# zzzxxxttt/SimpleDepthEstimation

Measured on AMD Instinct MI355X. Metric: training images/sec at 192x640 bs=12/GPU, higher is better.
Workload: dtype bf16; 1 GPU; Supervised ResNet-50 (BASELINE configs[1]), bf16 storage / fp32 accumulate, bs=12/GPU, 192x640, fwd+bwd+optimizer, random-init weights; global_batch=12, parallelism=dp1, hip_graph=True, allreduce_overlap=False

## Files before the change

include/sde_hip.h:

```cpp
#ifndef SDE_HIP_H
#define SDE_HIP_H
#include <stddef.h>
#include <stdint.h>

#ifdef __cplusplus
extern "C" {
#endif

typedef void* sde_stream_t;

#define SDE_MAX_CTX 4
#define SDE_F32 0
#define SDE_BF16 1
#define SDE_F16 2

#define SDE_REDUCE_ROWS 32

#define SDE_RESIZE_BILINEAR_AC 0
#define SDE_RESIZE_NEAREST 1

const char* sde_last_error(void);
int sde_version(void);

int sde_mark_time(uint64_t* slot, sde_stream_t stream);
// ... 22 lines not shown
    float ssim_w, C1, C2;
    const float* clip_thr;
} sde_photo_desc;

int sde_photo_num_blocks(int B, int h, int w, int backward);

int sde_photo_fwd(const sde_photo_desc* d, float* const* sampled, uint8_t* sel, float* maps, float* partial, float* loss_out,
                  float loss_scale, int accumulate, sde_stream_t stream);

int sde_photo_bwd(const sde_photo_desc* d, const float* const* sampled, const uint8_t* sel, const float* gout, float gscale, float* d_depth,
                  int accumulate_depth, float* pose_partial, float* const* d_pose, int accumulate_pose, sde_stream_t stream);
int sde_photo_multi_fwd(const sde_photo_desc* d, int n, float* const* sampled, uint8_t* const* sel, float* const* partial, float* loss_out,
                        sde_stream_t stream);
int sde_photo_multi_bwd(const sde_photo_desc* d, int n, const float* const* sampled, const uint8_t* const* sel, const float* gout, float* const* d_depth,
                        float* const* pose_partial, float* const* d_pose, sde_stream_t stream);
int sde_photo_multi_pose_finalize(const sde_photo_desc* d, int n, const float* const* pose_partial, float* const* d_pose, sde_stream_t stream);

int sde_mono_loss_fwd(const sde_photo_desc* d, int n, const float* photo_w, const float* smooth_w, float* const* sampled, uint8_t* const* sel,
                      float* const* photo_partial, float* const* sm_mean_part, float* const* sm_dn, float* const* sm_loss_part, float* const* sm_s_part,
                      float* per_scale, float* totals, int* ticket, sde_stream_t stream);
int sde_mono_loss_bwd(const sde_photo_desc* d, int n, const float* photo_w, const float* smooth_w, const float* const* sampled, const uint8_t* const* sel,
                      const float* g_rec, const float* g_smooth, const float* const* sm_mean_part, const float* const* sm_dn, const float* const* sm_s_part,
                      float* const* d_depth, float* const* pose_partial, float* const* d_pose, sde_stream_t stream);
int sde_smooth_multi_bwd(const sde_photo_desc* d, int n, const float* smooth_w, const float* g_smooth, const float* const* sm_mean_part, const float* const* sm_dn,
                         const float* const* sm_s_part, float* const* d_depth, int accumulate, sde_stream_t stream);

int sde_ssim_fwd(const float* x, const float* y, int B, int C, int H, int W, float C1, float C2, float* out, sde_stream_t stream);
int sde_ssim_bwd(const float* x, const float* y, const float* gout, int B, int C, int H, int W, float C1, float C2, float* coef_ws, float* dx, float* dy,
                 sde_stream_t stream);

int sde_smooth_num_blocks(int B, int h, int w);
int sde_smooth_fwd(const float* depth, const float* img, int B, int h, int w, float* mean_part, float* dn, float* loss_part, float* s_part,
                   float* loss_out, float loss_scale, int accumulate, sde_stream_t stream);
int sde_smooth_bwd(const float* depth, const float* dn, const float* mean_part, const float* s_part, const float* gout, float gscale, int B,
                   int h, int w, float* d_depth, int accumulate, sde_stream_t stream);

int sde_silog_num_blocks(int B, int h, int w);
int sde_silog_fwd(const float* est, const float* gt, int B, int h, int w, int H, int W, float variance_focus, float* part, float* stats,
                  sde_stream_t stream);
int sde_silog_bwd(const float* est, const float* gt, const float* stats, const float* gout, float gscale, float variance_focus, int B, int h,
                  int w, int H, int W, float* d_est, int accumulate, sde_stream_t stream);
#define SDE_SILOG_MAX_SCALES 4
int sde_silog_multi_num_blocks(int B, const int* h, const int* w, int n);
int sde_silog_multi_fwd(const float* const* est, const float* gt, int B, const int* h, const int* w, const float* weight, int n, int H, int W,
                        float variance_focus, float* part, float* stats, float* total, sde_stream_t stream);
int sde_silog_multi_bwd(const float* const* est, const float* gt, const float* stats, const float* gout, float gscale, float variance_focus, int B,
                        const int* h, const int* w, const float* weight, int n, int H, int W, float* const* d_est, sde_stream_t stream);

#define SDE_SRC_PLAIN 0
#define SDE_SRC_UPCAT 1
#define SDE_SRC_ZEROINS 2
#define SDE_ACT_NONE 0
#define SDE_ACT_ELU 1
#define SDE_ACT_RELU 2

typedef struct sde_conv_desc {
    const void* x0;
    const void* x1;
    int32_t dtype;
    int32_t C0, C1, H0, W0, IH, IW, src_mode;
    int32_t KH, KW, stride, pad;
    int32_t reflect;
    int32_t Bn, OH, OW;
} sde_conv_desc;

int sde_pack_weight(const float* w, void* out, int dtype, int Cout, int Cin, int KH, int KW, int Cin_pad, int Cout_pad, int for_dgrad,
                    sde_stream_t stream);

typedef struct sde_pack_item {
    const float* src;
    void* dst_fwd;
    void* dst_dgrad;
    int32_t Cout, Cin, KH, KW, Cin_pad, Cout_pad;
    int32_t src_layout, reserved;
    int64_t end;
} sde_pack_item;
#define SDE_W_OIHW 0
#define SDE_W_OHWI 1
int sde_pack_item_blocks(int Cout_pad, int Cin_pad, int KH, int KW);
int sde_pack_weights_batched(const sde_pack_item* items_dev, int n, long total_blocks, int dtype, sde_stream_t stream);

int sde_conv_fwd(const sde_conv_desc* d, const void* w_packed, const float* bias, int act, void* y, int Cout, int ldy, float* stats,
                 sde_stream_t stream);
size_t sde_conv_fwd_ws_bytes(const sde_conv_desc* d, int ldy);
int sde_conv_fwd_ws(const sde_conv_desc* d, const void* w_packed, const float* bias, int act, void* y, int Cout, int ldy, float* stats, void* ws,
                    size_t ws_bytes, sde_stream_t stream);
int sde_conv_dgrad_bnbwd_rows(const sde_conv_desc* d, int Cout, int ldy);
int sde_conv_dgrad_bnbwd(const sde_conv_desc* d, const void* w_packed, void* gm, int Cout, int ldy, const void* bn_y, const float* bnp, float* part,
                         sde_stream_t stream);
int sde_conv_dgrad_bnbwd_res_rows(const sde_conv_desc* d, int Cout, int ldy);
int sde_conv_dgrad_bnbwd_res(const sde_conv_desc* d, const void* w_packed, void* gm, int Cout, int ldy, const void* bn_y, const float* bnp, float* part,
                             const void* res_grad, const void* bn_out, sde_stream_t stream);
int sde_conv_fwd_tiles_m(const sde_conv_desc* d, int ldy);
int sde_conv_fwd_variant(const sde_conv_desc* d, int ldy);
int sde_conv_set_halo_min_blocks(int min_blocks);
#define SDE_OPT_PGEMM 1
#define SDE_OPT_PGEMM_DEPTH 2
#define SDE_OPT_PGEMM_3X3 3
#define SDE_OPT_PGEMM_TILE 4
#define SDE_OPT_SPLITK 5
#define SDE_OPT_WGRAD_BLOCKS 6
#define SDE_OPT_WGRAD_HALO 7
#define SDE_OPT_CONV_SMALL 8
#define SDE_OPT_WGRAD_DMA 9
#define SDE_OPT_BNBWD_FUSE 10
#define SDE_OPT_CU_RESERVE 11
#define SDE_OPT_WGRAD_DMA_RING 12
#define SDE_OPT_PGEMM_PER_CU 13
int sde_conv_set_option(int key, int value);
#define SDE_KERNEL_PGEMM 1
#define SDE_KERNEL_WGRAD_DMA 2
#define SDE_KERNEL_WGRAD_HALO 3
#define SDE_KERNEL_WGRAD_STAGED 4
#define SDE_KERNEL_WGRAD_SUM 5
#define SDE_KERNEL_WGRAD_REDUCE 6
int sde_kernel_lds_bytes(int kind, int variant);

#define SDE_WGRAD_FOLD_ROWS 16
int sde_conv_wgrad_splits(const sde_conv_desc* d, int Cout);
#define SDE_WGRAD_HALO_KERNEL 1
#define SDE_WGRAD_DMA_KERNEL 2
#define SDE_WGRAD_STAGED_KERNEL 3
int sde_conv_wgrad_variant(const sde_conv_desc* d, int Cout, int ldd);
int sde_conv_wgrad(const sde_conv_desc* d, const void* dy, int Cout, int ldd, int Cin_real, float* slab, int splits, float* dw, int accumulate,
                   sde_stream_t stream);

int sde_conv_wgrad_partial(const sde_conv_desc* d, const void* dy, int Cout, int ldd, float* slab, int splits, sde_stream_t stream);
typedef struct sde_wreduce_item {
    const float* slab;
    float* dw;
    int32_t rows , Cout, KHW, Cin_pad, Cin_real;
    int32_t accumulate;
} sde_wreduce_item;
#define SDE_WREDUCE_ACCUMULATE 1
#define SDE_WREDUCE_OHWI 2
int sde_wgrad_reduce_batched(const sde_wreduce_item* items, int n, sde_stream_t stream);

int sde_prep_input(const float* img, const float* mean, const float* std_, int B, int C, int H, int W, int Cpad, int flip, int dtype, void* out,
                   sde_stream_t stream);

int sde_bn_finalize(const float* part, int tiles, int C, long count, const float* gamma, const float* beta, float* running_mean, float* running_var,
                    float momentum, float eps, float* bnp, sde_stream_t stream);
int sde_bn_eval_params(const float* gamma, const float* beta, const float* running_mean, const float* running_var, float eps, int C, float* bnp,
                       sde_stream_t stream);
int sde_bn_apply(const void* y, const float* bnp, const void* residual, int relu, long M, int C, int dtype, void* out, sde_stream_t stream);
int sde_bn_finalize_apply_ok(int tiles, int C, int dtype);
int sde_bn_set_fuse(int on);
int sde_bn_finalize_apply(const float* part, int tiles, int C, long count, const float* gamma, const float* beta, float* running_mean, float* running_var,
                          float momentum, float eps, float* bnp, const void* y, const void* residual, int relu, int dtype, void* out, sde_stream_t stream);
int sde_reduce_num_blocks(long M, int C);
int sde_bn_bwd(const void* dout, const void* dout1, const void* dout2, const void* out, const void* y, const float* bnp, const float* gamma, int relu,
               long M, int C, int dtype, float* part, float* coef, float* dgamma, float* dbeta, int accumulate_params, void* gm, void* dy,
               sde_stream_t stream);
int sde_bn_bwd_from_part(const float* part, int rows, const void* gm, const void* y, const float* bnp, long M, int C, int dtype, float* coef,
                         float* dgamma, float* dbeta, int accumulate_params, void* dy, sde_stream_t stream);

int sde_maxpool_fwd(const void* x, int B, int H, int W, int C, int dtype, void* out, uint8_t* idx, sde_stream_t stream);
int sde_maxpool_bwd(const void* dout, const uint8_t* idx, int B, int H, int W, int C, int dtype, void* dx, sde_stream_t stream);
int sde_maxpool_bwd_sum(const void* dout, const void* dout1, const uint8_t* idx, int B, int H, int W, int C, int dtype, void* dx, sde_stream_t stream);

int sde_act_bwd_bias(const void* dout, const void* out, int act, long M, int C, int dtype, void* dz, float* part, float* dbias, int Cbias, int accumulate,
                     sde_stream_t stream);
int sde_act_bwd_bias_sum(const void* dout, const void* dout1, const void* out, int act, long M, int C, int dtype, void* dz, float* part, float* dbias, int Cbias,
                         int accumulate, sde_stream_t stream);
typedef struct sde_colsum_item {
    const float* part;
    float* out;
    int32_t rows, ld, C, accumulate;
} sde_colsum_item;
int sde_colsum_finalize_batched(const sde_colsum_item* items, int n, sde_stream_t stream);

int sde_refl_fold(const void* dxp, int B, int H, int W, int C, int C0, int upcat, int dtype, void* dx0, void* dx1, sde_stream_t stream);

int sde_depth_head_fwd(const void* y, int B, int H, int W, int ld, float min_depth, float max_depth, int flip, int dtype, float* depth, sde_stream_t stream);
int sde_depth_head_bwd(const void* y, const float* ddepth, int B, int H, int W, int ld, float min_depth, float max_depth, int flip, int dtype, void* dy,
                       sde_stream_t stream);
int sde_depth_head_bias_blocks(int B, int H, int W);
int sde_depth_head_bwd_bias(const void* y, const float* ddepth, int B, int H, int W, int ld, float min_depth, float max_depth, int flip, int dtype, void* dy,
                            float* part, float* dbias, int accumulate, sde_stream_t stream);

#define SDE_GN_CHUNKS 64
int sde_gn_relu_fwd(const void* x, const float* gamma, const float* beta, int B, int HW, int C, int G, float eps, int relu, int dtype, float* part, float* gnp,
                    void* out, sde_stream_t stream);
int sde_gn_relu_bwd(const void* dout, const void* out, const void* x, const float* gnp, const float* gamma, int B, int HW, int C, int G, int relu, int dtype,
                    float* part, float* coef, float* dgamma, float* dbeta, int accumulate_params, void* dx, sde_stream_t stream);
int sde_gn_relu_res_fwd(const void* x, const void* res, const float* gamma, const float* beta, int B, int HW, int C, int G, float eps, int relu, int dtype,
                        float* part, float* gnp, void* out, sde_stream_t stream);
int sde_gn_relu_res_bwd(const void* dout, const void* out, const void* x, const void* res, const float* gnp, const float* gamma, int B, int HW, int C, int G, int relu,
                        int dtype, float* part, float* coef, float* dgamma, float* dbeta, int accumulate_params, void* dx, sde_stream_t stream);

int sde_dilate_split(const void* x, int B, int H, int W, int C, int d, int dtype, void* out, sde_stream_t stream);
int sde_dilate_merge(const void* sub, int B, int H, int W, int C, int d, int dtype, void* out, sde_stream_t stream);
int sde_upsample2_fwd(const void* x, int B, int H, int W, int C, int dtype, void* out, sde_stream_t stream);
int sde_upsample2_bwd(const void* dout, int B, int H, int W, int C, int dtype, void* dx, sde_stream_t stream);
#define SDE_CAT_MAX 6
typedef struct sde_cat_piece {
    void* p;
    int32_t C, ld, f32map, reserved;
} sde_cat_piece;
int sde_cat_fwd(const sde_cat_piece* pieces, int n, long P, int Ct, int dtype, void* out, sde_stream_t stream);
int sde_cat_bwd(const void* dout, long P, int Ct, int dtype, const sde_cat_piece* grads, int n, sde_stream_t stream);
#define SDE_STATS_ROWS 256
int sde_channel_stats_tiles(long M);
int sde_channel_stats(const void* x, long M, int C, int dtype, float* part, sde_stream_t stream);
int sde_relu_fwd(const void* x, long n, int dtype, void* y, sde_stream_t stream);
int sde_lpg_fwd(const void* y, int B, int h, int w, int ld, int r, float max_depth, int ds, int dtype, float* full, float* down, sde_stream_t stream);
int sde_lpg_bwd(const void* y, const float* dfull, const float* ddown, int B, int h, int w, int ld, int r, float max_depth, int ds, int dtype, void* dy,
                sde_stream_t stream);
int sde_sigmoid_head_fwd(const void* y, int B, int H, int W, int ld, float scale, const float* focal, float focal_div, int flip, int dtype, float* out,
                         sde_stream_t stream);
int sde_sigmoid_head_bwd(const void* y, const float* dout, int B, int H, int W, int ld, float scale, const float* focal, float focal_div, int flip, int dtype,
                         void* dy, sde_stream_t stream);


#define SDE_RLN_CHUNKS 32
int sde_randln_chunks(int HW);
int sde_randln_fwd(const void* y, const void* res, const float* gamma, const float* beta, const float* z, const float* stddev, int train, int B, int HW,
                   int C, int Cr, float eps, int relu, int dtype, float* part, float* rlnp, void* out, sde_stream_t stream);
int sde_randln_bwd(const void* d0, const void* d1, const void* d2, const void* out, const void* y, const float* rlnp, const float* gamma, int relu, int B,
                   int HW, int C, int Cr, int dtype, float* part, float* dgamma, float* dbeta, int accumulate, void* gm, void* dx, sde_stream_t stream);
int sde_bilinear2_fwd(const void* x, int B, int H, int W, int C, int dtype, void* out, sde_stream_t stream);
int sde_bilinear2_bwd(const void* dout, int B, int H, int W, int C, int dtype, void* dx, sde_stream_t stream);
int sde_softplus_head_fwd(const void* y, int B, int H, int W, int ld, int flip, int dtype, float* out, sde_stream_t stream);
int sde_softplus_head_bwd(const void* y, const float* dout, int B, int H, int W, int ld, int flip, int dtype, void* dy, sde_stream_t stream);

int sde_deconv3x3s2_fwd(const void* x, const void* w_packed, const float* bias, int act, int B, int H, int W, int C, int Cout, int ldy, int dtype,
                        void* y, sde_stream_t stream);

int sde_gconv3x3_stats_rows(int B, int H, int W, int C, int G, int stride, int dtype);
int sde_gconv3x3_fwd(const void* x, const float* w, int w_ohwi, int B, int H, int W, int C, int G, int stride, int dtype, void* y, float* stats,
                     sde_stream_t stream);
int sde_gconv3x3_dgrad(const void* dz, const float* w, int w_ohwi, int B, int H, int W, int C, int G, int stride, int dtype, void* dx,
                       sde_stream_t stream);
size_t sde_gconv3x3_wgrad_ws_bytes(int B, int H, int W, int C, int G, int stride, int dtype);
int sde_gconv3x3_wgrad(const void* x, const void* dz, int B, int H, int W, int C, int G, int stride, int dtype, float* ws, size_t ws_bytes, float* dw,
                       int flags, sde_stream_t stream);

int sde_motion_resize_cat_fwd(const float* field, int h, int w, const void* skip, int B, int H, int W, int Cs, int Cr, int Cx, int dtype, void* X,
                              float* up, sde_stream_t stream);
int sde_motion_resize_cat_bwd(const void* dX0, const void* dX1, const float* dup, int B, int H, int W, int Cx, int Cr, int Cs, int h, int w, int dtype,
                              float* dfield, void* dskip, sde_stream_t stream);
int sde_motion_tail_fwd(const void* o1, const void* o2, const float* w3, const float* up, long P, int ld, int mid, int dtype, float* out,
                        sde_stream_t stream);
int sde_motion_tail_blocks(long P, int ld, int dtype);
int sde_motion_tail_bwd(const float* dout, const void* o1, const void* o2, const float* w3, long P, int ld, int mid, int dtype, void* do1, void* do2,
                        float* part, float* dw3, sde_stream_t stream);
int sde_motion_head_blocks(long P);
int sde_motion_head_fwd(const float* field, const float* scale, const float* weight, int mask, int B, int H, int W, float* part, unsigned char* keep,
                        float* out, sde_stream_t stream);
int sde_motion_head_bwd(const float* dout, const float* field, const float* scale, const float* weight, const unsigned char* keep, int B, int H, int W,
                        float* dfield, float* part, sde_stream_t stream);
int sde_prep_input_bwd(const void* d0, const void* d1, int B, int C, int H, int W, int Cp, int dtype, float* dimg, sde_stream_t stream);

int sde_conv3d_fwd(const void* x, const float* w, const float* bias, int B, int H, int W, int D, int dtype, void* y, sde_stream_t stream);
int sde_conv3d_dgrad(const void* dy, const float* w, int B, int H, int W, int D, int dtype, void* dx, sde_stream_t stream);
int sde_conv3d_wgrad_num_blocks(int B, int H, int W, int D, int dtype);
int sde_conv3d_wgrad(const void* x, const void* dy, int B, int H, int W, int D, int dtype, float* part, float* dw, float* dbias, int accumulate,
                     sde_stream_t stream);

int sde_space_to_depth(const void* x, int B, int H, int W, int C, int dtype, void* y, sde_stream_t stream);
int sde_depth_to_space(const void* x, int B, int H, int W, int C4, int dtype, void* y, sde_stream_t stream);
int sde_concat_fwd(const void* p0, const void* p1, const float* inv, int add, int B, int H, int W, int C0, int C1, int Ct, int dtype, void* out,
                   sde_stream_t stream);
int sde_concat_bwd(const void* dout, int add, int B, int H, int W, int C0, int C1, int Ct, int dtype, void* d0, void* d1, float* d_inv, sde_stream_t stream);
int sde_inv_depth_head_fwd(const void* y, int B, int H, int W, int ld, float min_depth_head, float min_depth, float max_depth, int flip, int dtype, float* inv,
                           float* depth, sde_stream_t stream);
int sde_inv_depth_head_bwd(const void* y, const float* d_inv, const float* d_depth, int B, int H, int W, int ld, float min_depth_head, float min_depth,
                           float max_depth, int flip, int dtype, void* dy, sde_stream_t stream);

#define SDE_ADAM_MAX_SEG 8
#define SDE_GRAD_NORM_WORK 1024
typedef struct sde_adam_desc {
    long seg_end[SDE_ADAM_MAX_SEG];
    float seg_lr[SDE_ADAM_MAX_SEG], seg_wd[SDE_ADAM_MAX_SEG];
    int32_t nseg, decoupled_wd;
    float beta1, beta2, eps, bias_corr1, bias_corr2, grad_scale;
    const float* scale_state;
    double beta1_d, beta2_d;
    const float* clip_state;
} sde_adam_desc;
int sde_adam_step(float* p, const float* g, float* m, float* v, long n, const sde_adam_desc* d, sde_stream_t stream);
int sde_grad_check(const float* g, long n, float* scale_state, sde_stream_t stream);
int sde_grad_norm(const float* g, long n, float* work, float* clip_state, float grad_scale, float max_norm, sde_stream_t stream);
int sde_loss_scale_update(float* scale_state, float growth_factor, float backoff_factor, int growth_interval, sde_stream_t stream);


int sde_image_prep_u8(const uint8_t* src, int N, int Hs, int Ws, int h, int w, const int* xtab, const int* ytab, const float* jit, unsigned* lsum, float* img,
                      float* orig, sde_stream_t stream);
int sde_image_prep_u8_multi(const uint8_t* const* src, int G, int N, int Hs, int Ws, int h, int w, const int* xtab, const int* ytab, const float* jit, unsigned* lsum,
                            float* const* img, float* const* orig, sde_stream_t stream);

#define SDE_EVAL_NSUM 11
int sde_depth_metrics_num_blocks(int crop_h, int crop_w);
int sde_depth_metrics(const float* pred, int ph, int pw, const float* gt, int gh, int gw, const int* ymap, const int* xmap, int y0, int y1,
                      int x0, int x1, float min_depth, float max_depth, int gt_scale, double* part, float* med, unsigned* keys, double* out,
                      sde_stream_t stream);

int sde_depth_present(const float* pred, int N, int ph, int pw, const int* ymap, const int* xmap, int H, int W, float vmax, float gamma,
                      const uint8_t* lut, const uint8_t* frame, float* depth_full, uint16_t* depth_u16, uint8_t* canvas, sde_stream_t stream);

typedef struct sde_rgbd_desc {
    const float *frame_A, *frame_B, *depth_A, *depth_B, *K, *R, *t;
    int32_t N, H, W, ssim;
    float C1, C2;
} sde_rgbd_desc;
int sde_view_synthesis_pp(const float* img, const float* depth, const float* K, const float* R, const float* t, int B, int C, int H, int W, float* sampled,
// ... 52 lines not shown
```

simpledepthestimation_amd/csrc/nn.hip:

```cpp
#include <stdlib.h>
#include "common.h"
#include "sde_hip.h"

namespace {

template <typename T> struct VecOf;
template <> struct VecOf<float> { static constexpr int V = 4; };
template <> struct VecOf<bf16_t> { static constexpr int V = 8; };
template <> struct VecOf<half_t> { static constexpr int V = 8; };

template <typename T> __device__ __forceinline__ void load_vec(const T* p, float* v);
template <> __device__ __forceinline__ void load_vec<float>(const float* p, float* v) {
    const float4 t = *reinterpret_cast<const float4*>(p);
    v[0] = t.x; v[1] = t.y; v[2] = t.z; v[3] = t.w;
}
template <> __device__ __forceinline__ void load_vec<bf16_t>(const bf16_t* p, float* v) {
    const uint4 t = *reinterpret_cast<const uint4*>(p);
    const uint32_t w[4] = {t.x, t.y, t.z, t.w};
#pragma unroll
    for (int i = 0; i < 4; ++i) {
        v[2 * i] = __uint_as_float(w[i] << 16);
        v[2 * i + 1] = __uint_as_float(w[i] & 0xffff0000u);
    }
}
template <> __device__ __forceinline__ void load_vec<half_t>(const half_t* p, float* v) {
    typedef __attribute__((ext_vector_type(8))) _Float16 h8;
    const h8 t = *reinterpret_cast<const h8*>(p);
#pragma unroll
    for (int i = 0; i < 8; ++i) v[i] = (float)t[i];
}
template <typename T> __device__ __forceinline__ void store_vec(T* p, const float* v);
template <> __device__ __forceinline__ void store_vec<float>(float* p, const float* v) {
    *reinterpret_cast<float4*>(p) = make_float4(v[0], v[1], v[2], v[3]);
}
template <> __device__ __forceinline__ void store_vec<bf16_t>(bf16_t* p, const float* v) {
    bf16_t o[8];
#pragma unroll
    for (int i = 0; i < 8; ++i) o[i] = (bf16_t)v[i];
    *reinterpret_cast<uint4*>(p) = *reinterpret_cast<uint4*>(o);
}

template <> __device__ __forceinline__ void store_vec<half_t>(half_t* p, const float* v) {
    typedef __attribute__((ext_vector_type(8))) _Float16 h8;
    h8 o;
#pragma unroll
    for (int i = 0; i < 8; ++i) o[i] = (_Float16)v[i];
    *reinterpret_cast<h8*>(p) = o;
}

template <typename T>
__global__ void __launch_bounds__(256) prep_input_kernel(const float* __restrict__ img, const float* __restrict__ mean, const float* __restrict__ std_,
                                                         int B, int C, int H, int W, int Cpad, int flip, T* __restrict__ out) {
    const long n = (long)B * H * W;
    for (long i = (long)blockIdx.x * 256 + threadIdx.x; i < n; i += (long)gridDim.x * 256) {
        const int x = (int)(i % W), y = (int)((i / W) % H), b = (int)(i / ((long)W * H));
        const int xs = flip ? W - 1 - x : x;
        T* o = out + i * Cpad;
        for (int c = 0; c < Cpad; ++c) {
            float v = 0.f;
            if (c < C) {
                v = img[(((long)b * C + c) * H + y) * W + xs];
                if (mean) v = (v - mean[c]) / std_[c];
            }
            o[c] = (T)v;
        }
    }
}

__global__ void __launch_bounds__(1024) rows_reduce_kernel(const float* __restrict__ in, int rows, int width, int chunk, float* __restrict__ out) {
    __shared__ float sh[16][64];
    const int col = blockIdx.x * 64 + (threadIdx.x & 63), sub = threadIdx.x >> 6, ro = blockIdx.y;
    const int r0 = ro * chunk, r1 = min(rows, r0 + chunk);
    float s = 0.f;
    if (col < width)
        for (int r = r0 + sub; r < r1; r += 16) s += in[(size_t)r * width + col];
    sh[sub][threadIdx.x & 63] = s;
    __syncthreads();
    if (sub == 0 && col < width) {
        float t = 0.f;
#pragma unroll
        for (int i = 0; i < 16; ++i) t += sh[i][threadIdx.x & 63];
        out[(size_t)ro * width + col] = t;
    }
}

__device__ __forceinline__ double half_wave_sum(double v) {
#pragma unroll
    for (int o = 16; o > 0; o >>= 1) v += __shfl_xor(v, o, 64);
    return v;
}

constexpr int SLAB_T = 1024, SLAB_RL = SLAB_T / 16, SLAB_RES = SLAB_RL * 17, SLAB_SH = SLAB_RES + 16;
__device__ __forceinline__ void slab_colsum16(const float* __restrict__ part, int rows, int width, int col0, double* sh ) {
    const int rl = threadIdx.x >> 4, e = threadIdx.x & 15;
    const bool ok = col0 + e < width;
    const float* src = part + col0 + e;
    double a0 = 0, a1 = 0, a2 = 0, a3 = 0;
    int t = rl;
    if (ok) {
        for (; t + 7 * SLAB_RL < rows; t += 8 * SLAB_RL) {
            float v[8];
#pragma unroll
            for (int i = 0; i < 8; ++i) v[i] = src[(size_t)(t + i * SLAB_RL) * width];
            a0 += (double)v[0] + (double)v[4]; a1 += (double)v[1] + (double)v[5]; a2 += (double)v[2] + (double)v[6]; a3 += (double)v[3] + (double)v[7];
        }
        for (; t + 3 * SLAB_RL < rows; t += 4 * SLAB_RL) {
            const float v0 = src[(size_t)t * width], v1 = src[(size_t)(t + SLAB_RL) * width], v2 = src[(size_t)(t + 2 * SLAB_RL) * width],
                        v3 = src[(size_t)(t + 3 * SLAB_RL) * width];
            a0 += v0; a1 += v1; a2 += v2; a3 += v3;
        }
        for (; t < rows; t += SLAB_RL) a0 += src[(size_t)t * width];
    }
    sh[rl * 17 + e] = (a0 + a1) + (a2 + a3);
    __syncthreads();
    if (threadIdx.x < 16) {
        double tot = 0;
        for (int i = 0; i < SLAB_RL; ++i) tot += sh[i * 17 + threadIdx.x];
        sh[SLAB_RES + threadIdx.x] = tot;
    }
    __syncthreads();
}

__global__ void __launch_bounds__(SLAB_T) bn_finalize_kernel(const float* __restrict__ part, int tiles, int C, float count, const float* __restrict__ gamma,
                                                          const float* __restrict__ beta, float* __restrict__ rmean, float* __restrict__ rvar,
                                                          float momentum, float eps, float* __restrict__ bnp) {
    __shared__ double sh[SLAB_SH];
    slab_colsum16(part, tiles, 2 * C, blockIdx.x * 16, sh);
    const int c = blockIdx.x * 8 + threadIdx.x;
    if (threadIdx.x >= 8 || c >= C) return;
    const double s1 = sh[SLAB_RES + 2 * threadIdx.x], s2 = sh[SLAB_RES + 2 * threadIdx.x + 1];
    const double mean = s1 / count;
    double var = s2 / count - mean * mean;
    if (var < 0) var = 0;
    const float rstd = (float)(1.0 / sqrt(var + (double)eps));
    const float sc = gamma[c] * rstd;
    bnp[c] = (float)mean; bnp[C + c] = rstd; bnp[2 * C + c] = sc; bnp[3 * C + c] = beta[c] - (float)mean * sc;
    if (rmean) {
        const double unb = count > 1.f ? var * count / (count - 1.0) : var;
        rmean[c] = (1.f - momentum) * rmean[c] + momentum * (float)mean;
        rvar[c] = (1.f - momentum) * rvar[c] + momentum * (float)unb;
    }
}

__global__ void __launch_bounds__(64) bn_eval_params_kernel(const float* __restrict__ gamma, const float* __restrict__ beta,
                                                            const float* __restrict__ rmean, const float* __restrict__ rvar, float eps, int C,
                                                            float* __restrict__ bnp) {
    const int c = blockIdx.x * 64 + threadIdx.x;
    if (c >= C) return;
    const float rstd = 1.0f / sqrtf(rvar[c] + eps);
    const float sc = gamma[c] * rstd;
    bnp[c] = rmean[c]; bnp[C + c] = rstd; bnp[2 * C + c] = sc; bnp[3 * C + c] = beta[c] - rmean[c] * sc;
}

template <typename T>
__global__ void __launch_bounds__(256) bn_apply_kernel(const T* __restrict__ y, const float* __restrict__ bnp, const T* __restrict__ res, int relu,
                                                       long M, int C, T* __restrict__ out) {
    constexpr int V = VecOf<T>::V;
    const int cch = C / V;
    const long total = M * cch;
    for (long i = (long)blockIdx.x * 256 + threadIdx.x; i < total; i += (long)gridDim.x * 256) {
        const int c0 = (int)(i % cch) * V;
        float v[V], r[V];
        load_vec<T>(y + i * V, v);
        if (res) load_vec<T>(res + i * V, r);
#pragma unroll
        for (int e = 0; e < V; ++e) {
            float t = fmaf(v[e], bnp[2 * C + c0 + e], bnp[3 * C + c0 + e]);
            if (res) t += r[e];
            if (relu) t = fmaxf(t, 0.f);
            v[e] = t;
        }
        store_vec<T>(out + i * V, v);
    }
}

constexpr int BNFA_MAX_ROWS = 256;
template <typename T>
__global__ void __launch_bounds__(256) bn_finalize_apply_kernel(const float* __restrict__ part, int rows, int C, float count, const float* __restrict__ gamma,
                                                                const float* __restrict__ beta, float* __restrict__ rmean, float* __restrict__ rvar,
                                                                float momentum, float eps, float* __restrict__ bnp, const T* __restrict__ y,
                                                                const T* __restrict__ res, int relu, long M, long rows_per_wg, T* __restrict__ out) {
    constexpr int V = VecOf<T>::V;
    __shared__ double acc[8][128];
    __shared__ float ss[2][64];
    const int strip = blockIdx.x, c0 = strip * 64;
    const int tid = threadIdx.x;
    {
        const int f4 = tid & 31, rl = tid >> 5;
        const float4* src = reinterpret_cast<const float4*>(part + (size_t)c0 * 2) + f4;
        const size_t ld4 = (size_t)C / 2;
        double a[4] = {0, 0, 0, 0}, b[4] = {0, 0, 0, 0};
        int r = rl;
        for (; r + 56 < rows; r += 64) {
            float4 v[8];
#pragma unroll
            for (int i = 0; i < 8; ++i) v[i] = src[(size_t)(r + 8 * i) * ld4];
#pragma unroll
            for (int i = 0; i < 8; i += 2) {
                a[0] += v[i].x; a[1] += v[i].y; a[2] += v[i].z; a[3] += v[i].w;
                b[0] += v[i + 1].x; b[1] += v[i + 1].y; b[2] += v[i + 1].z; b[3] += v[i + 1].w;
            }
        }
        for (; r < rows; r += 8) { const float4 v = src[(size_t)r * ld4]; a[0] += v.x; a[1] += v.y; a[2] += v.z; a[3] += v.w; }
#pragma unroll
        for (int e = 0; e < 4; ++e) acc[rl][f4 * 4 + e] = a[e] + b[e];
    }
    __syncthreads();
    if (tid < 64) {
        const int c = c0 + tid;
        double s1 = 0, s2 = 0;
#pragma unroll
        for (int i = 0; i < 8; ++i) { s1 += acc[i][2 * tid]; s2 += acc[i][2 * tid + 1]; }
        const double mean = s1 / count;
        double var = s2 / count - mean * mean;
        if (var < 0) var = 0;
        const float rstd = (float)(1.0 / sqrt(var + (double)eps));
        const float sc = gamma[c] * rstd, sf = beta[c] - (float)mean * sc;
        ss[0][tid] = sc; ss[1][tid] = sf;
        if (blockIdx.y == 0) {
            bnp[c] = (float)mean; bnp[C + c] = rstd; bnp[2 * C + c] = sc; bnp[3 * C + c] = sf;
            if (rmean) {
                const double unb = count > 1.f ? var * count / (count - 1.0) : var;
                rmean[c] = (1.f - momentum) * rmean[c] + momentum * (float)mean;
                rvar[c] = (1.f - momentum) * rvar[c] + momentum * (float)unb;
            }
        }
    }
    __syncthreads();
    const int g8 = tid & 7, rl = tid >> 3;
    float sc[V], sf[V];
#pragma unroll
    for (int e = 0; e < V; ++e) { sc[e] = ss[0][g8 * V + e]; sf[e] = ss[1][g8 * V + e]; }
    const long r0 = (long)blockIdx.y * rows_per_wg, r1 = min(M, r0 + rows_per_wg);
    for (long r = r0 + rl; r < r1; r += 32) {
        const long off = r * C + c0 + g8 * V;
        float v[V], rr[V];
        load_vec<T>(y + off, v);
        if (res) load_vec<T>(res + off, rr);
#pragma unroll
        for (int e = 0; e < V; ++e) {
            float t = fmaf(v[e], sc[e], sf[e]);
            if (res) t += rr[e];
            if (relu) t = fmaxf(t, 0.f);
            v[e] = t;
        }
        store_vec<T>(out + off, v);
    }
}

template <int NV, int NT = 256>
__device__ __forceinline__ void block_group_reduce(float (&a)[NV], int cch, float* sh) {
    const int t = threadIdx.x;
#pragma unroll
    for (int e = 0; e < NV; ++e) sh[e * NT + t] = a[e];
    __syncthreads();
    if (NT > 256) {
        if (t < 256) {
            for (int r = t + 256; r < NT; r += 256)
#pragma unroll
                for (int e = 0; e < NV; ++e) a[e] += sh[e * NT + r];
#pragma unroll
            for (int e = 0; e < NV; ++e) sh[e * NT + t] = a[e];
        }
        __syncthreads();
    }
    if (t < cch) {
        for (int r = t + cch; r < 256; r += cch)
#pragma unroll
            for (int e = 0; e < NV; ++e) a[e] += sh[e * NT + r];
    }
}

template <typename T, int V>
__device__ __forceinline__ void round_vec(float* d) {
    if (sizeof(T) == 4) return;
#pragma unroll
    for (int e = 0; e < V; ++e) d[e] = (float)(T)d[e];
}

template <typename T, int V>
__device__ __forceinline__ void bn_load_dz(const T* d0, const T* d1, const T* d2, const T* out, int relu, long off, float* d, const float* yv,
                                           const float* sc, const float* sf) {
    load_vec<T>(d0 + off, d);
    if (d1) {
        float t[V];
        load_vec<T>(d1 + off, t);
#pragma unroll
        for (int e = 0; e < V; ++e) d[e] += t[e];
    }
    if (d2) {
        float t[V];
        load_vec<T>(d2 + off, t);
#pragma unroll
        for (int e = 0; e < V; ++e) d[e] += t[e];
    }
    if (relu == 1) {
        float o[V];
        load_vec<T>(out + off, o);
#pragma unroll
        for (int e = 0; e < V; ++e) d[e] = o[e] > 0.f ? d[e] : 0.f;
    } else if (relu == 2) {
#pragma unroll
        for (int e = 0; e < V; ++e) d[e] = fmaf(yv[e], sc[e], sf[e]) > 0.f ? d[e] : 0.f;
    }
}

template <typename T, int NT = 256>
__global__ void __launch_bounds__(NT) bn_bwd_reduce_kernel(const T* __restrict__ dout, const T* __restrict__ dout1, const T* __restrict__ dout2,
                                                           const T* __restrict__ out, const T* __restrict__ y,
                                                           const float* __restrict__ bnp, int relu, long M, int C, long rows_per_block,
                                                           float* __restrict__ part, T* __restrict__ gm) {
    constexpr int V = VecOf<T>::V;
    extern __shared__ float sh[];
    const int cch = C / V;
    if (NT > 256 || (cch <= 256 && 256 % cch == 0)) {
        const int col = threadIdx.x % cch, c0 = col * V;
        float mean[V], rstd[V], sc[V], sf[V], acc[2 * V];
#pragma unroll
        for (int e = 0; e < V; ++e) {
            mean[e] = bnp[c0 + e]; rstd[e] = bnp[C + c0 + e]; sc[e] = bnp[2 * C + c0 + e]; sf[e] = bnp[3 * C + c0 + e];
            acc[e] = 0.f; acc[V + e] = 0.f;
        }
        const long total = M * cch;
        for (long i = (long)blockIdx.x * NT + threadIdx.x; i < total; i += (long)gridDim.x * NT) {
            float d[V], yv[V];
            load_vec<T>(y + i * V, yv);
            bn_load_dz<T, V>(dout, dout1, dout2, out, relu, i * V, d, yv, sc, sf);
            if (gm) {
                round_vec<T, V>(d);
                store_vec<T>(gm + i * V, d);
            }
#pragma unroll
            for (int e = 0; e < V; ++e) { acc[e] += d[e]; acc[V + e] += d[e] * ((yv[e] - mean[e]) * rstd[e]); }
        }
        block_group_reduce<2 * V, NT>(acc, cch, sh);
        if (threadIdx.x < cch) {
#pragma unroll
            for (int e = 0; e < V; ++e) {
                part[((size_t)blockIdx.x * C + c0 + e) * 2] = acc[e];
                part[((size_t)blockIdx.x * C + c0 + e) * 2 + 1] = acc[V + e];
            }
        }
        return;
    }
    for (int i = threadIdx.x; i < 2 * C; i += 256) sh[i] = 0.f;
    __syncthreads();
    const long r0 = (long)blockIdx.x * rows_per_block, r1 = min(M, r0 + rows_per_block);
    const long total = (r1 - r0) * cch;
    for (long i = threadIdx.x; i < total; i += 256) {
        const int col = (int)(i % cch), c0 = col * V;
        const long off = (r0 * cch + i) * V;
        float d[V], yv[V];
        load_vec<T>(y + off, yv);
        bn_load_dz<T, V>(dout, dout1, dout2, out, relu, off, d, yv, bnp + 2 * C + c0, bnp + 3 * C + c0);
        if (gm) {
            round_vec<T, V>(d);
            store_vec<T>(gm + off, d);
        }
#pragma unroll
        for (int e = 0; e < V; ++e) {
            const float xh = (yv[e] - bnp[c0 + e]) * bnp[C + c0 + e];
            atomicAdd(&sh[c0 + e], d[e]); atomicAdd(&sh[C + c0 + e], d[e] * xh);
        }
    }
    __syncthreads();
    for (int i = threadIdx.x; i < C; i += 256) {
        part[((size_t)blockIdx.x * C + i) * 2] = sh[i];
        part[((size_t)blockIdx.x * C + i) * 2 + 1] = sh[C + i];
    }
}

__global__ void __launch_bounds__(SLAB_T) bn_bwd_finalize_kernel(const float* __restrict__ part, int nblk, int C, float count, float* __restrict__ dgamma,
                                                              float* __restrict__ dbeta, int accumulate, float* __restrict__ coef) {
    __shared__ double sh[SLAB_SH];
    slab_colsum16(part, nblk, 2 * C, blockIdx.x * 16, sh);
    const int c = blockIdx.x * 8 + threadIdx.x;
    if (threadIdx.x >= 8 || c >= C) return;
    const double s1 = sh[SLAB_RES + 2 * threadIdx.x], s2 = sh[SLAB_RES + 2 * threadIdx.x + 1];
    coef[c] = (float)(s1 / count); coef[C + c] = (float)(s2 / count);
    dgamma[c] = accumulate ? dgamma[c] + (float)s2 : (float)s2;
    dbeta[c] = accumulate ? dbeta[c] + (float)s1 : (float)s1;
}

template <typename T>
__global__ void __launch_bounds__(256) bn_bwd_apply_kernel(const T* __restrict__ dz_in, const T* __restrict__ y,
                                                           const float* __restrict__ bnp, const float* __restrict__ coef, long M, int C,
                                                           T* __restrict__ dy) {
    constexpr int V = VecOf<T>::V;
    const int cch = C / V;
    const long total = M * cch;
    for (long i = (long)blockIdx.x * 256 + threadIdx.x; i < total; i += (long)gridDim.x * 256) {
        const int c0 = (int)(i % cch) * V;
        float d[V], yv[V], g[V];
        load_vec<T>(dz_in + i * V, d);
        load_vec<T>(y + i * V, yv);
#pragma unroll
        for (int e = 0; e < V; ++e) {
            const float xh = (yv[e] - bnp[c0 + e]) * bnp[C + c0 + e];
            g[e] = bnp[2 * C + c0 + e] * (d[e] - coef[c0 + e] - xh * coef[C + c0 + e]);
        }
        store_vec<T>(dy + i * V, g);
    }
}

template <typename T>
__global__ void __launch_bounds__(256) bn_bwd_finalize_apply_kernel(const float* __restrict__ part, int rows, int C, float count, float* __restrict__ dgamma,
                                                                    float* __restrict__ dbeta, int accumulate, const T* __restrict__ dz_in,
                                                                    const T* __restrict__ y, const float* __restrict__ bnp, long M, long rows_per_wg,
                                                                    T* __restrict__ dy) {
    constexpr int V = VecOf<T>::V;
    __shared__ double acc[8][128];
    __shared__ float cf[2][64];
    const int c0 = blockIdx.x * 64, tid = threadIdx.x;
    {
        const int f4 = tid & 31, rl = tid >> 5;
        const float4* src = reinterpret_cast<const float4*>(part + (size_t)c0 * 2) + f4;
        const size_t ld4 = (size_t)C / 2;
        double a[4] = {0, 0, 0, 0}, b[4] = {0, 0, 0, 0};
        int r = rl;
        for (; r + 56 < rows; r += 64) {
            float4 v[8];
#pragma unroll
            for (int i = 0; i < 8; ++i) v[i] = src[(size_t)(r + 8 * i) * ld4];
#pragma unroll
            for (int i = 0; i < 8; i += 2) {
                a[0] += v[i].x; a[1] += v[i].y; a[2] += v[i].z; a[3] += v[i].w;
                b[0] += v[i + 1].x; b[1] += v[i + 1].y; b[2] += v[i + 1].z; b[3] += v[i + 1].w;
            }
        }
        for (; r < rows; r += 8) { const float4 v = src[(size_t)r * ld4]; a[0] += v.x; a[1] += v.y; a[2] += v.z; a[3] += v.w; }
#pragma unroll
        for (int e = 0; e < 4; ++e) acc[rl][f4 * 4 + e] = a[e] + b[e];
    }
    __syncthreads();
    if (tid < 64) {
        const int c = c0 + tid;
        double s1 = 0, s2 = 0;
#pragma unroll
        for (int i = 0; i < 8; ++i) { s1 += acc[i][2 * tid]; s2 += acc[i][2 * tid + 1]; }
        cf[0][tid] = (float)(s1 / count); cf[1][tid] = (float)(s2 / count);
        if (blockIdx.y == 0) {
            dgamma[c] = accumulate ? dgamma[c] + (float)s2 : (float)s2;
            dbeta[c] = accumulate ? dbeta[c] + (float)s1 : (float)s1;
        }
    }
    __syncthreads();
    const int g8 = tid & 7, rl = tid >> 3;
    float mean[V], rstd[V], sc[V], k1[V], k2[V];
#pragma unroll
    for (int e = 0; e < V; ++e) {
        const int c = c0 + g8 * V + e;
        mean[e] = bnp[c]; rstd[e] = bnp[C + c]; sc[e] = bnp[2 * C + c]; k1[e] = cf[0][g8 * V + e]; k2[e] = cf[1][g8 * V + e];
    }
    const long r0 = (long)blockIdx.y * rows_per_wg, r1 = min(M, r0 + rows_per_wg);
    for (long r = r0 + rl; r < r1; r += 32) {
        const long off = r * C + c0 + g8 * V;
        float d[V], yv[V], g[V];
        load_vec<T>(dz_in + off, d);
        load_vec<T>(y + off, yv);
#pragma unroll
        for (int e = 0; e < V; ++e) {
            const float xh = (yv[e] - mean[e]) * rstd[e];
            g[e] = sc[e] * (d[e] - k1[e] - xh * k2[e]);
        }
        store_vec<T>(dy + off, g);
    }
}

template <typename T>
__global__ void __launch_bounds__(256) maxpool_fwd_kernel(const T* __restrict__ x, int B, int H, int W, int C, int OH, int OW, T* __restrict__ out,
                                                          uint8_t* __restrict__ idx) {
    constexpr int V = VecOf<T>::V;
    const int cch = C / V;
    const long total = (long)B * OH * OW * cch;
    for (long i = (long)blockIdx.x * 256 + threadIdx.x; i < total; i += (long)gridDim.x * 256) {
        const int col = (int)(i % cch);
        const long pix = i / cch;
        const int ow = (int)(pix % OW), oh = (int)((pix / OW) % OH), b = (int)(pix / ((long)OW * OH));
        float best[V]; int bi[V];
#pragma unroll
        for (int e = 0; e < V; ++e) { best[e] = -INFINITY; bi[e] = 0; }
#pragma unroll
        for (int kh = 0; kh < 3; ++kh) {
            const int ih = oh * 2 - 1 + kh;
            if (ih < 0 || ih >= H) continue;
#pragma unroll
            for (int kw = 0; kw < 3; ++kw) {
                const int iw = ow * 2 - 1 + kw;
                if (iw < 0 || iw >= W) continue;
                float v[V];
                load_vec<T>(x + (((long)b * H + ih) * W + iw) * C + col * V, v);
#pragma unroll
                for (int e = 0; e < V; ++e)
                    if (v[e] > best[e] || v[e] != v[e]) { best[e] = v[e]; bi[e] = kh * 3 + kw; }
            }
        }
        store_vec<T>(out + i * V, best);
        uint8_t* ip = idx + i * V;
#pragma unroll
        for (int e = 0; e < V; ++e) ip[e] = (uint8_t)bi[e];
    }
}

template <typename T>
__global__ void __launch_bounds__(256) maxpool_bwd_kernel(const T* __restrict__ dout, const T* __restrict__ dout1, const uint8_t* __restrict__ idx, int B, int H,
                                                          int W, int C, int OH, int OW, T* __restrict__ dx) {
    constexpr int V = VecOf<T>::V;
    const int cch = C / V;
    const long total = (long)B * H * W * cch;
    for (long i = (long)blockIdx.x * 256 + threadIdx.x; i < total; i += (long)gridDim.x * 256) {
        const int col = (int)(i % cch);
        const long pix = i / cch;
        const int iw = (int)(pix % W), ih = (int)((pix / W) % H), b = (int)(pix / ((long)W * H));
        float g[V];
#pragma unroll
        for (int e = 0; e < V; ++e) g[e] = 0.f;
#pragma unroll
        for (int kh = 0; kh < 3; ++kh) {
            const int t = ih + 1 - kh;
            if (t < 0 || (t & 1)) continue;
            const int oh = t >> 1;
            if (oh >= OH) continue;
#pragma unroll
            for (int kw = 0; kw < 3; ++kw) {
                const int u = iw + 1 - kw;
                if (u < 0 || (u & 1)) continue;
                const int ow = u >> 1;
                if (ow >= OW) continue;
                const long o = ((((long)b * OH + oh) * OW + ow) * cch + col) * V;
                float d[V];
                load_vec<T>(dout + o, d);
                if (dout1) {
                    float t[V];
                    load_vec<T>(dout1 + o, t);
#pragma unroll
                    for (int e = 0; e < V; ++e) d[e] += t[e];
                }
                const uint8_t* ip = idx + o;
#pragma unroll
                for (int e = 0; e < V; ++e)
                    if (ip[e] == kh * 3 + kw) g[e] += d[e];
            }
        }
        store_vec<T>(dx + i * V, g);
    }
}

template <typename T>
__global__ void __launch_bounds__(256) act_bwd_bias_kernel(const T* __restrict__ dout, const T* __restrict__ dout1, const T* __restrict__ out, int act, long M,
                                                           int C, long rows_per_block, T* __restrict__ dz, float* __restrict__ part) {
    constexpr int V = VecOf<T>::V;
    extern __shared__ float sh[];
    const int cch = C / V;
    if (cch <= 256 && 256 % cch == 0) {
        const int col = threadIdx.x % cch, c0 = col * V;
        float acc[V];
#pragma unroll
        for (int e = 0; e < V; ++e) acc[e] = 0.f;
        const long total = M * cch;
        const long stride = (long)gridDim.x * 256;
        long i = (long)blockIdx.x * 256 + threadIdx.x;
        for (; i + 3 * stride < total; i += 4 * stride) {
            float d[4][V], o[4][V];
#pragma unroll
            for (int u = 0; u < 4; ++u) load_vec<T>(dout + (i + u * stride) * V, d[u]);
            if (dout1) {
#pragma unroll
                for (int u = 0; u < 4; ++u) load_vec<T>(dout1 + (i + u * stride) * V, o[u]);
#pragma unroll
                for (int u = 0; u < 4; ++u)
#pragma unroll
                    for (int e = 0; e < V; ++e) d[u][e] += o[u][e];
            }
            if (act != SDE_ACT_NONE) {
#pragma unroll
                for (int u = 0; u < 4; ++u) load_vec<T>(out + (i + u * stride) * V, o[u]);
#pragma unroll
                for (int u = 0; u < 4; ++u)
#pragma unroll
                    for (int e = 0; e < V; ++e) {
                        if (act == SDE_ACT_ELU) d[u][e] = o[u][e] > 0.f ? d[u][e] : d[u][e] * (o[u][e] + 1.0f);
                        else d[u][e] = o[u][e] > 0.f ? d[u][e] : 0.f;
                    }
            }
#pragma unroll
            for (int u = 0; u < 4; ++u) {
                if (dz) store_vec<T>(dz + (i + u * stride) * V, d[u]);
#pragma unroll
                for (int e = 0; e < V; ++e) acc[e] += d[u][e];
            }
        }
        for (; i < total; i += stride) {
            float d[V], o[V];
            load_vec<T>(dout + i * V, d);
            if (dout1) {
                load_vec<T>(dout1 + i * V, o);
#pragma unroll
                for (int e = 0; e < V; ++e) d[e] += o[e];
            }
            if (act != SDE_ACT_NONE) {
                load_vec<T>(out + i * V, o);
#pragma unroll
                for (int e = 0; e < V; ++e) {
                    if (act == SDE_ACT_ELU) d[e] = o[e] > 0.f ? d[e] : d[e] * (o[e] + 1.0f);
                    else d[e] = o[e] > 0.f ? d[e] : 0.f;
                }
            }
            if (dz) store_vec<T>(dz + i * V, d);
#pragma unroll
            for (int e = 0; e < V; ++e) acc[e] += d[e];
        }
        if (part) {
            block_group_reduce<V>(acc, cch, sh);
            if (threadIdx.x < cch)
#pragma unroll
                for (int e = 0; e < V; ++e) part[(size_t)blockIdx.x * C + c0 + e] = acc[e];
        }
        return;
    }
    if (part) {
        for (int i = threadIdx.x; i < C; i += 256) sh[i] = 0.f;
        __syncthreads();
    }
    const long r0 = (long)blockIdx.x * rows_per_block, r1 = min(M, r0 + rows_per_block);
    const long total = (r1 - r0) * cch;
    for (long i = threadIdx.x; i < total; i += 256) {
        const int c0 = (int)(i % cch) * V;
        const long off = (r0 * cch + i) * V;
        float d[V], o[V];
        load_vec<T>(dout + off, d);
        if (dout1) {
            load_vec<T>(dout1 + off, o);
#pragma unroll
            for (int e = 0; e < V; ++e) d[e] += o[e];
        }
        if (act != SDE_ACT_NONE) {
            load_vec<T>(out + off, o);
#pragma unroll
            for (int e = 0; e < V; ++e) {
                if (act == SDE_ACT_ELU) d[e] = o[e] > 0.f ? d[e] : d[e] * (o[e] + 1.0f);
                else if (act == SDE_ACT_RELU) d[e] = o[e] > 0.f ? d[e] : 0.f;
            }
        }
        if (dz) store_vec<T>(dz + off, d);
        if (part) {
#pragma unroll
            for (int e = 0; e < V; ++e) atomicAdd(&sh[c0 + e], d[e]);
        }
    }
    if (part) {
        __syncthreads();
        for (int i = threadIdx.x; i < C; i += 256) part[(size_t)blockIdx.x * C + i] = sh[i];
    }
}

__global__ void __launch_bounds__(SLAB_T) colsum_finalize_kernel(const float* __restrict__ part, int nblk, int ld, int C, float* __restrict__ out, int accumulate) {
    __shared__ double sh[SLAB_SH];
    slab_colsum16(part, nblk, ld, blockIdx.x * 16, sh);
    const int c = blockIdx.x * 16 + threadIdx.x;
    if (threadIdx.x >= 16 || c >= C) return;
    const double sv = sh[SLAB_RES + threadIdx.x];
    out[c] = accumulate ? out[c] + (float)sv : (float)sv;
}

constexpr int COLSUM_MAX_ITEMS = 64;
struct ColsumBatch {
    const float* part[COLSUM_MAX_ITEMS];
    float* out[COLSUM_MAX_ITEMS];
    int rows[COLSUM_MAX_ITEMS], ld[COLSUM_MAX_ITEMS], C[COLSUM_MAX_ITEMS], accumulate[COLSUM_MAX_ITEMS];
    int first[COLSUM_MAX_ITEMS + 1];
    int n;
};
__global__ void __launch_bounds__(SLAB_T) colsum_finalize_batched_kernel(const ColsumBatch b) {
    __shared__ double sh[SLAB_SH];
    int k = 0;
    while (k + 1 < b.n && (int)blockIdx.x >= b.first[k + 1]) ++k;
    const int col0 = ((int)blockIdx.x - b.first[k]) * 16;
    slab_colsum16(b.part[k], b.rows[k], b.ld[k], col0, sh);
    const int c = col0 + threadIdx.x;
    if (threadIdx.x >= 16 || c >= b.C[k]) return;
    const double sv = sh[SLAB_RES + threadIdx.x];
    float* out = b.out[k];
    out[c] = b.accumulate[k] ? out[c] + (float)sv : (float)sv;
}

template <typename T>
__device__ __forceinline__ void fold_at(const T* __restrict__ dxp, int b, int h, int w, int H, int W, int C, int c0, float* g) {
    constexpr int V = VecOf<T>::V;
#pragma unroll
    for (int e = 0; e < V; ++e) g[e] = 0.f;
    int hs[3], ws[3], nh = 0, nw = 0;
    hs[nh++] = h + 1;
    if (h == 1) hs[nh++] = 0;
    if (h == H - 2) hs[nh++] = H + 1;
    ws[nw++] = w + 1;
    if (w == 1) ws[nw++] = 0;
    if (w == W - 2) ws[nw++] = W + 1;
// ... 367 lines not shown
            s2 += part[((size_t)q * C + c) * 2 + 1];
        }
        s1 = wave_sum_f64(s1); s2 = wave_sum_f64(s2);
        if (threadIdx.x == 0) {
            dgamma[c] = accumulate ? dgamma[c] + (float)s2 : (float)s2;
            dbeta[c] = accumulate ? dbeta[c] + (float)s1 : (float)s1;
        }
    }
}

template <typename T>
__global__ void __launch_bounds__(256) gn_bwd_apply_kernel(const T* __restrict__ dout, const T* __restrict__ out, const T* __restrict__ x, const T* __restrict__ res,
                                                           const float* __restrict__ gnp, const float* __restrict__ coef, const float* __restrict__ gamma,
                                                           int B, int HW, int C, int G, int relu, T* __restrict__ dx) {
    constexpr int V = VecOf<T>::V;
    const int cch = C / V, cpg = C / G;
    const long total = (long)B * HW * cch;
    for (long i = (long)blockIdx.x * 256 + threadIdx.x; i < total; i += (long)gridDim.x * 256) {
        const int c0 = (int)(i % cch) * V, b = (int)(i / ((long)HW * cch));
        float d[V], o[V], xv[V];
        load_vec<T>(dout + i * V, d);
        if (relu) load_vec<T>(out + i * V, o);
        load_vec<T>(x + i * V, xv);
        if (res) {
            float rr[V];
            load_vec<T>(res + i * V, rr);
#pragma unroll
            for (int e = 0; e < V; ++e) xv[e] += rr[e];
        }
#pragma unroll
        for (int e = 0; e < V; ++e) {
            const size_t gi = ((size_t)b * G + (c0 + e) / cpg) * 2;
            float de = d[e];
            if (relu) de = gn_act_grad(de, o[e], relu);
            const float xh = (xv[e] - gnp[gi]) * gnp[gi + 1];
            d[e] = gnp[gi + 1] * (gamma[c0 + e] * de - coef[gi] - xh * coef[gi + 1]);
        }
        store_vec<T>(dx + i * V, d);
    }
}

__global__ void __launch_bounds__(256) adam_kernel(float* __restrict__ p, const float* __restrict__ g, float* __restrict__ m, float* __restrict__ v, long n,
                                                   const sde_adam_desc d) {
    float gs = d.grad_scale;
    float bc1 = d.bias_corr1, bc2 = d.bias_corr2;
    if (d.scale_state) {
        if (d.scale_state[1] != 0.f) return;
        gs /= d.scale_state[0];
        const double t = (double)d.scale_state[3] + 1.0;
        bc1 = (float)(1.0 - pow(d.beta1_d, t));
        bc2 = (float)(1.0 - pow(d.beta2_d, t));
    }
    if (d.clip_state) gs *= d.clip_state[1];
    const float beta1 = d.beta1, beta2 = d.beta2, rbc2 = 1.0f / sqrtf(bc2);
    for (long i = (long)blockIdx.x * 256 + threadIdx.x; i < n; i += (long)gridDim.x * 256) {
        int s = 0;
        while (s < d.nseg - 1 && i >= d.seg_end[s]) ++s;
        const float lr = d.seg_lr[s], wd = d.seg_wd[s];
        float gi = g[i] * gs, pi = p[i];
        if (d.decoupled_wd) pi *= (1.0f - lr * wd);
        else gi += wd * pi;
        const float mi = beta1 * m[i] + (1.0f - beta1) * gi;
        const float vi = beta2 * v[i] + (1.0f - beta2) * gi * gi;
        m[i] = mi; v[i] = vi;
        const float denom = sqrtf(vi) * rbc2 + d.eps;
        p[i] = pi - (lr / bc1) * (mi / denom);
    }
}

__global__ void __launch_bounds__(256) grad_check_kernel(const float4* __restrict__ g4, long n4, const float* __restrict__ tail, int ntail, float* __restrict__ state) {
    bool bad = false;
    for (long i = (long)blockIdx.x * 256 + threadIdx.x; i < n4; i += (long)gridDim.x * 256) {
        const float4 q = g4[i];
        const float t = fabsf(q.x) + fabsf(q.y) + fabsf(q.z) + fabsf(q.w);
        bad |= !(t <= 3.0e38f);
    }
    if (blockIdx.x == 0 && (int)threadIdx.x < ntail) bad |= !(fabsf(tail[threadIdx.x]) <= 3.0e38f);
    if (__any(bad) && (threadIdx.x & 63) == 0) state[1] = 1.0f;
}

__global__ void loss_scale_update_kernel(float* __restrict__ state, float growth, float backoff, int interval) {
    if (threadIdx.x != 0 || blockIdx.x != 0) return;
    if (state[1] != 0.f) { state[0] *= backoff; state[2] = 0.f; }
    else {
        state[3] += 1.f;
        const float t = state[2] + 1.f;
        if (t >= (float)interval) { state[0] *= growth; state[2] = 0.f; } else state[2] = t;
    }
    state[1] = 0.f;
}

__global__ void __launch_bounds__(256) grad_norm_partial_kernel(const float4* __restrict__ g4, long n4, const float* __restrict__ tail, int ntail, float* __restrict__ work) {
    __shared__ float red[16];
    float sx = 0.f, sy = 0.f, sz = 0.f, sw = 0.f;
    for (long i = (long)blockIdx.x * 256 + threadIdx.x; i < n4; i += (long)gridDim.x * 256) {
        const float4 q = g4[i];
        sx = fmaf(q.x, q.x, sx); sy = fmaf(q.y, q.y, sy); sz = fmaf(q.z, q.z, sz); sw = fmaf(q.w, q.w, sw);
    }
    float s = (sx + sy) + (sz + sw);
    if (blockIdx.x == 0 && (int)threadIdx.x < ntail) s = fmaf(tail[threadIdx.x], tail[threadIdx.x], s);
    s = sde_block_sum(s, red);
    if (threadIdx.x == 0) work[blockIdx.x] = s;
}

__global__ void __launch_bounds__(256) grad_norm_finalize_kernel(const float* __restrict__ work, int nwork, float grad_scale, float max_norm, float* __restrict__ clip_state) {
    __shared__ float red[16];
    float s = 0.f;
    for (int i = threadIdx.x; i < nwork; i += 256) s += work[i];
    s = sde_block_sum(s, red);
    if (threadIdx.x == 0) {
        const float total = grad_scale * sqrtf(s);
        float coef = max_norm / (total + 1e-6f);
        if (coef > 1.0f) coef = 1.0f;
        clip_state[0] = total;
        clip_state[1] = coef;
    }
}

const float* pre_reduce(const float* part, int& rows, int width, hipStream_t s) {
    constexpr int thr = 4096;
    if (rows <= thr) return part;
    float* out = const_cast<float*>(part) + (size_t)rows * width;
    const int chunk = (rows + SDE_REDUCE_ROWS - 1) / SDE_REDUCE_ROWS;
    const int rows_out = (rows + chunk - 1) / chunk;
    hipLaunchKernelGGL(rows_reduce_kernel, dim3((width + 63) / 64, rows_out), dim3(1024), 0, s, part, rows, width, chunk, out);
    rows = rows_out;
    return out;
}

int grid_for(long n_items) {
    long nb = (n_items + 255) / 256;
    if (nb < 1) nb = 1;
    if (nb > 8192) nb = 8192;
    return (int)nb;
}

}

#define DISPATCH_T(dtype, CALL_F32, CALL_BF16, CALL_F16) \
    do {                                        \
        if ((dtype) == SDE_BF16) { CALL_BF16; }  \
        else if ((dtype) == SDE_F16) { CALL_F16; } \
        else { CALL_F32; }                      \
    } while (0)

extern "C" {

int sde_prep_input(const float* img, const float* mean, const float* std_, int B, int C, int H, int W, int Cpad, int flip, int dtype, void* out,
                   sde_stream_t stream) {
    SDE_CHECK_ARG(img && out && B > 0 && C > 0 && H > 0 && W > 0 && Cpad >= C, "sde_prep_input: bad argument");
    SDE_CHECK_ARG((mean == nullptr) == (std_ == nullptr), "sde_prep_input: mean/std must both be given or both be null");
    hipStream_t s = (hipStream_t)stream;
    const int nb = grid_for((long)B * H * W);
    DISPATCH_T(dtype, hipLaunchKernelGGL(prep_input_kernel<float>, dim3(nb), dim3(256), 0, s, img, mean, std_, B, C, H, W, Cpad, flip, (float*)out),
               hipLaunchKernelGGL(prep_input_kernel<bf16_t>, dim3(nb), dim3(256), 0, s, img, mean, std_, B, C, H, W, Cpad, flip, (bf16_t*)out),
               hipLaunchKernelGGL(prep_input_kernel<half_t>, dim3(nb), dim3(256), 0, s, img, mean, std_, B, C, H, W, Cpad, flip, (half_t*)out));
    SDE_CHECK_LAUNCH("sde_prep_input");
    return SDE_OK;
}

int sde_bn_finalize(const float* part, int tiles, int C, long count, const float* gamma, const float* beta, float* running_mean, float* running_var,
                    float momentum, float eps, float* bnp, sde_stream_t stream) {
    SDE_CHECK_ARG(part && gamma && beta && bnp && tiles > 0 && C > 0 && count > 0, "sde_bn_finalize: bad argument");
    int rows = tiles;
    const float* src = pre_reduce(part, rows, 2 * C, (hipStream_t)stream);
    hipLaunchKernelGGL(bn_finalize_kernel, dim3(sde_cdiv(C, 8)), dim3(SLAB_T), 0, (hipStream_t)stream, src, rows, C, (float)count, gamma, beta, running_mean,
                       running_var, momentum, eps, bnp);
    SDE_CHECK_LAUNCH("sde_bn_finalize");
    return SDE_OK;
}

static int g_bn_fuse = 1;
static int g_bn_wide = 1;
int sde_bn_set_fuse(int on) {
    const int old = g_bn_fuse ? (g_bn_wide ? 1 : 2) : 0;
    g_bn_fuse = on ? 1 : 0;
    g_bn_wide = on == 1;
    return old;
}

int sde_bn_finalize_apply_ok(int tiles, int C, int dtype) { return SDE_IS16(dtype) && C % 64 == 0 && tiles >= 1 && tiles <= BNFA_MAX_ROWS; }

int sde_bn_finalize_apply(const float* part, int tiles, int C, long count, const float* gamma, const float* beta, float* running_mean, float* running_var,
                          float momentum, float eps, float* bnp, const void* y, const void* residual, int relu, int dtype, void* out, sde_stream_t stream) {
    SDE_CHECK_ARG(part && gamma && beta && bnp && y && out && count > 0, "sde_bn_finalize_apply: bad argument");
    SDE_CHECK_ARG(sde_bn_finalize_apply_ok(tiles, C, dtype), "sde_bn_finalize_apply: needs a 16-bit type, C %% 64 == 0 and <= %d slab rows (tiles=%d C=%d)",
                  BNFA_MAX_ROWS, tiles, C);
    const long M = count;
    const int strips = C / 64;
    long chunks = (1024 + strips - 1) / strips;
    long rpw = (M + chunks - 1) / chunks;
    rpw = (rpw + 31) / 32 * 32;
    if (rpw < 32) rpw = 32;
    chunks = (M + rpw - 1) / rpw;
    const dim3 grid((unsigned)strips, (unsigned)chunks);
    hipStream_t s = (hipStream_t)stream;
    if (dtype == SDE_BF16)
        hipLaunchKernelGGL(bn_finalize_apply_kernel<bf16_t>, grid, dim3(256), 0, s, part, tiles, C, (float)count, gamma, beta, running_mean, running_var, momentum, eps,
                           bnp, (const bf16_t*)y, (const bf16_t*)residual, relu, M, rpw, (bf16_t*)out);
    else
        hipLaunchKernelGGL(bn_finalize_apply_kernel<half_t>, grid, dim3(256), 0, s, part, tiles, C, (float)count, gamma, beta, running_mean, running_var, momentum, eps,
                           bnp, (const half_t*)y, (const half_t*)residual, relu, M, rpw, (half_t*)out);
    SDE_CHECK_LAUNCH("sde_bn_finalize_apply");
    return SDE_OK;
}

int sde_bn_eval_params(const float* gamma, const float* beta, const float* running_mean, const float* running_var, float eps, int C, float* bnp,
                       sde_stream_t stream) {
    SDE_CHECK_ARG(gamma && beta && running_mean && running_var && bnp && C > 0, "sde_bn_eval_params: bad argument");
    hipLaunchKernelGGL(bn_eval_params_kernel, dim3(sde_cdiv(C, 64)), dim3(64), 0, (hipStream_t)stream, gamma, beta, running_mean, running_var, eps, C, bnp);
    SDE_CHECK_LAUNCH("sde_bn_eval_params");
    return SDE_OK;
}

int sde_bn_apply(const void* y, const float* bnp, const void* residual, int relu, long M, int C, int dtype, void* out, sde_stream_t stream) {
    const int V = SDE_IS16(dtype) ? 8 : 4;
    SDE_CHECK_ARG(y && bnp && out && M > 0 && C > 0 && C % V == 0, "sde_bn_apply: bad argument (C=%d)", C);
    hipStream_t s = (hipStream_t)stream;
    const int nb = grid_for(M * (C / V));
    DISPATCH_T(dtype, hipLaunchKernelGGL(bn_apply_kernel<float>, dim3(nb), dim3(256), 0, s, (const float*)y, bnp, (const float*)residual, relu, M, C, (float*)out),
               hipLaunchKernelGGL(bn_apply_kernel<bf16_t>, dim3(nb), dim3(256), 0, s, (const bf16_t*)y, bnp, (const bf16_t*)residual, relu, M, C, (bf16_t*)out),
               hipLaunchKernelGGL(bn_apply_kernel<half_t>, dim3(nb), dim3(256), 0, s, (const half_t*)y, bnp, (const half_t*)residual, relu, M, C, (half_t*)out));
    SDE_CHECK_LAUNCH("sde_bn_apply");
    return SDE_OK;
}

int sde_reduce_num_blocks(long M, int C) {
    constexpr long cap = 1024;
    long nb = (M * (long)C / 8 + 1023) / 1024;
    if (nb > cap) nb = cap;
    if (nb < 1) nb = 1;
    return (int)nb;
}

int sde_bn_bwd(const void* dout, const void* dout1, const void* dout2, const void* out, const void* y, const float* bnp, const float* gamma, int relu,
               long M, int C, int dtype, float* part, float* coef, float* dgamma, float* dbeta, int accumulate_params, void* gm, void* dy,
               sde_stream_t stream) {
    const int V = SDE_IS16(dtype) ? 8 : 4;
    SDE_CHECK_ARG(dout && y && bnp && part && coef && dgamma && dbeta && dy && M > 0 && C > 0 && C % V == 0, "sde_bn_bwd: bad argument");
    if (relu && !out) relu = 2;
    SDE_CHECK_ARG(gm || (!relu && !dout1 && !dout2), "sde_bn_bwd: a masked or summed gradient needs the gm buffer");
    SDE_CHECK_ARG(dout1 || !dout2, "sde_bn_bwd: dout2 without dout1");
    (void)gamma;
    hipStream_t s = (hipStream_t)stream;
    int nblk = sde_reduce_num_blocks(M, C);
    const long rpb = (M + nblk - 1) / nblk;
    const size_t lds = (2 * (size_t)C > 256 * 16 ? 2 * (size_t)C : 256 * 16) * sizeof(float);
    const int cch = C / V;
    const bool wide = g_bn_fuse && g_bn_wide && SDE_IS16(dtype) && C % 64 == 0 && nblk > BNFA_MAX_ROWS && cch <= 256 && 256 % cch == 0;
    if (wide) {
        nblk = (nblk + 3) / 4;
        if (dtype == SDE_BF16)
            hipLaunchKernelGGL((bn_bwd_reduce_kernel<bf16_t, 1024>), dim3(nblk), dim3(1024), 1024 * 16 * sizeof(float), s, (const bf16_t*)dout, (const bf16_t*)dout1,
                               (const bf16_t*)dout2, (const bf16_t*)out, (const bf16_t*)y, bnp, relu, M, C, rpb, part, (bf16_t*)gm);
        else
            hipLaunchKernelGGL((bn_bwd_reduce_kernel<half_t, 1024>), dim3(nblk), dim3(1024), 1024 * 16 * sizeof(float), s, (const half_t*)dout, (const half_t*)dout1,
                               (const half_t*)dout2, (const half_t*)out, (const half_t*)y, bnp, relu, M, C, rpb, part, (half_t*)gm);
    } else
    DISPATCH_T(dtype,
               hipLaunchKernelGGL(bn_bwd_reduce_kernel<float>, dim3(nblk), dim3(256), lds, s, (const float*)dout, (const float*)dout1, (const float*)dout2, (const float*)out, (const float*)y, bnp, relu, M, C, rpb, part, (float*)gm),
               hipLaunchKernelGGL(bn_bwd_reduce_kernel<bf16_t>, dim3(nblk), dim3(256), lds, s, (const bf16_t*)dout, (const bf16_t*)dout1, (const bf16_t*)dout2, (const bf16_t*)out, (const bf16_t*)y, bnp, relu, M, C, rpb, part, (bf16_t*)gm),
               hipLaunchKernelGGL(bn_bwd_reduce_kernel<half_t>, dim3(nblk), dim3(256), lds, s, (const half_t*)dout, (const half_t*)dout1, (const half_t*)dout2, (const half_t*)out, (const half_t*)y, bnp, relu, M, C, rpb, part, (half_t*)gm));
    SDE_CHECK_LAUNCH("sde_bn_bwd/reduce");
    const void* dz = gm ? gm : dout;
    if (g_bn_fuse && SDE_IS16(dtype) && C % 64 == 0 && nblk <= BNFA_MAX_ROWS) {
        const int strips = C / 64;
        long chunks = (1024 + strips - 1) / strips;
        long rpw = (M + chunks - 1) / chunks;
        rpw = (rpw + 31) / 32 * 32;
        chunks = (M + rpw - 1) / rpw;
        const dim3 grid((unsigned)strips, (unsigned)chunks);
        if (dtype == SDE_BF16)
            hipLaunchKernelGGL(bn_bwd_finalize_apply_kernel<bf16_t>, grid, dim3(256), 0, s, part, nblk, C, (float)M, dgamma, dbeta, accumulate_params, (const bf16_t*)dz,
                               (const bf16_t*)y, bnp, M, rpw, (bf16_t*)dy);
        else
            hipLaunchKernelGGL(bn_bwd_finalize_apply_kernel<half_t>, grid, dim3(256), 0, s, part, nblk, C, (float)M, dgamma, dbeta, accumulate_params, (const half_t*)dz,
                               (const half_t*)y, bnp, M, rpw, (half_t*)dy);
        SDE_CHECK_LAUNCH("sde_bn_bwd/finalize+apply");
        return SDE_OK;
    }
    int rows = nblk;
    const float* src = pre_reduce(part, rows, 2 * C, s);
    hipLaunchKernelGGL(bn_bwd_finalize_kernel, dim3(sde_cdiv(C, 8)), dim3(SLAB_T), 0, s, src, rows, C, (float)M, dgamma, dbeta, accumulate_params, coef);
    SDE_CHECK_LAUNCH("sde_bn_bwd/finalize");
    const int nb = grid_for(M * (C / V));
    DISPATCH_T(dtype,
               hipLaunchKernelGGL(bn_bwd_apply_kernel<float>, dim3(nb), dim3(256), 0, s, (const float*)dz, (const float*)y, bnp, coef, M, C, (float*)dy),
               hipLaunchKernelGGL(bn_bwd_apply_kernel<bf16_t>, dim3(nb), dim3(256), 0, s, (const bf16_t*)dz, (const bf16_t*)y, bnp, coef, M, C, (bf16_t*)dy),
               hipLaunchKernelGGL(bn_bwd_apply_kernel<half_t>, dim3(nb), dim3(256), 0, s, (const half_t*)dz, (const half_t*)y, bnp, coef, M, C, (half_t*)dy));
    SDE_CHECK_LAUNCH("sde_bn_bwd/apply");
    return SDE_OK;
}

int sde_bn_bwd_from_part(const float* part, int rows, const void* gm, const void* y, const float* bnp, long M, int C, int dtype, float* coef,
                         float* dgamma, float* dbeta, int accumulate_params, void* dy, sde_stream_t stream) {
    const int V = SDE_IS16(dtype) ? 8 : 4;
    SDE_CHECK_ARG(part && gm && y && bnp && coef && dgamma && dbeta && dy && rows > 0 && M > 0 && C > 0 && C % V == 0, "sde_bn_bwd_from_part: bad argument");
    hipStream_t s = (hipStream_t)stream;
    if (g_bn_fuse && SDE_IS16(dtype) && C % 64 == 0 && rows <= BNFA_MAX_ROWS) {
        const int strips = C / 64;
        long chunks = (1024 + strips - 1) / strips;
        long rpw = (M + chunks - 1) / chunks;
        rpw = (rpw + 31) / 32 * 32;
        chunks = (M + rpw - 1) / rpw;
        const dim3 grid((unsigned)strips, (unsigned)chunks);
        if (dtype == SDE_BF16)
            hipLaunchKernelGGL(bn_bwd_finalize_apply_kernel<bf16_t>, grid, dim3(256), 0, s, part, rows, C, (float)M, dgamma, dbeta, accumulate_params, (const bf16_t*)gm,
                               (const bf16_t*)y, bnp, M, rpw, (bf16_t*)dy);
        else
            hipLaunchKernelGGL(bn_bwd_finalize_apply_kernel<half_t>, grid, dim3(256), 0, s, part, rows, C, (float)M, dgamma, dbeta, accumulate_params, (const half_t*)gm,
                               (const half_t*)y, bnp, M, rpw, (half_t*)dy);
        SDE_CHECK_LAUNCH("sde_bn_bwd_from_part/finalize+apply");
        return SDE_OK;
    }
    int r = rows;
    const float* src = pre_reduce(part, r, 2 * C, s);
    hipLaunchKernelGGL(bn_bwd_finalize_kernel, dim3(sde_cdiv(C, 8)), dim3(SLAB_T), 0, s, src, r, C, (float)M, dgamma, dbeta, accumulate_params, coef);
    SDE_CHECK_LAUNCH("sde_bn_bwd_from_part/finalize");
    const int nb = grid_for(M * (C / V));
    DISPATCH_T(dtype,
               hipLaunchKernelGGL(bn_bwd_apply_kernel<float>, dim3(nb), dim3(256), 0, s, (const float*)gm, (const float*)y, bnp, coef, M, C, (float*)dy),
               hipLaunchKernelGGL(bn_bwd_apply_kernel<bf16_t>, dim3(nb), dim3(256), 0, s, (const bf16_t*)gm, (const bf16_t*)y, bnp, coef, M, C, (bf16_t*)dy),
               hipLaunchKernelGGL(bn_bwd_apply_kernel<half_t>, dim3(nb), dim3(256), 0, s, (const half_t*)gm, (const half_t*)y, bnp, coef, M, C, (half_t*)dy));
    SDE_CHECK_LAUNCH("sde_bn_bwd_from_part/apply");
    return SDE_OK;
}

int sde_maxpool_fwd(const void* x, int B, int H, int W, int C, int dtype, void* out, uint8_t* idx, sde_stream_t stream) {
    const int V = SDE_IS16(dtype) ? 8 : 4;
    SDE_CHECK_ARG(x && out && idx && B > 0 && H > 1 && W > 1 && C % V == 0, "sde_maxpool_fwd: bad argument");
    const int OH = (H + 2 - 3) / 2 + 1, OW = (W + 2 - 3) / 2 + 1;
    hipStream_t s = (hipStream_t)stream;
    const int nb = grid_for((long)B * OH * OW * (C / V));
    DISPATCH_T(dtype, hipLaunchKernelGGL(maxpool_fwd_kernel<float>, dim3(nb), dim3(256), 0, s, (const float*)x, B, H, W, C, OH, OW, (float*)out, idx),
               hipLaunchKernelGGL(maxpool_fwd_kernel<bf16_t>, dim3(nb), dim3(256), 0, s, (const bf16_t*)x, B, H, W, C, OH, OW, (bf16_t*)out, idx),
               hipLaunchKernelGGL(maxpool_fwd_kernel<half_t>, dim3(nb), dim3(256), 0, s, (const half_t*)x, B, H, W, C, OH, OW, (half_t*)out, idx));
    SDE_CHECK_LAUNCH("sde_maxpool_fwd");
    return SDE_OK;
}

int sde_maxpool_bwd(const void* dout, const uint8_t* idx, int B, int H, int W, int C, int dtype, void* dx, sde_stream_t stream) {
    return sde_maxpool_bwd_sum(dout, nullptr, idx, B, H, W, C, dtype, dx, stream);
}

int sde_maxpool_bwd_sum(const void* dout, const void* dout1, const uint8_t* idx, int B, int H, int W, int C, int dtype, void* dx, sde_stream_t stream) {
    const int V = SDE_IS16(dtype) ? 8 : 4;
    SDE_CHECK_ARG(dout && idx && dx && B > 0 && H > 1 && W > 1 && C % V == 0, "sde_maxpool_bwd: bad argument");
    const int OH = (H + 2 - 3) / 2 + 1, OW = (W + 2 - 3) / 2 + 1;
    hipStream_t s = (hipStream_t)stream;
    const int nb = grid_for((long)B * H * W * (C / V));
    DISPATCH_T(dtype, hipLaunchKernelGGL(maxpool_bwd_kernel<float>, dim3(nb), dim3(256), 0, s, (const float*)dout, (const float*)dout1, idx, B, H, W, C, OH, OW, (float*)dx),
               hipLaunchKernelGGL(maxpool_bwd_kernel<bf16_t>, dim3(nb), dim3(256), 0, s, (const bf16_t*)dout, (const bf16_t*)dout1, idx, B, H, W, C, OH, OW, (bf16_t*)dx),
               hipLaunchKernelGGL(maxpool_bwd_kernel<half_t>, dim3(nb), dim3(256), 0, s, (const half_t*)dout, (const half_t*)dout1, idx, B, H, W, C, OH, OW, (half_t*)dx));
    SDE_CHECK_LAUNCH("sde_maxpool_bwd");
    return SDE_OK;
}

int sde_act_bwd_bias(const void* dout, const void* out, int act, long M, int C, int dtype, void* dz, float* part, float* dbias, int Cbias, int accumulate,
                     sde_stream_t stream) {
    return sde_act_bwd_bias_sum(dout, nullptr, out, act, M, C, dtype, dz, part, dbias, Cbias, accumulate, stream);
}

int sde_act_bwd_bias_sum(const void* dout, const void* dout1, const void* out, int act, long M, int C, int dtype, void* dz, float* part, float* dbias, int Cbias,
                         int accumulate, sde_stream_t stream) {
    const int V = SDE_IS16(dtype) ? 8 : 4;
    SDE_CHECK_ARG(dout && M > 0 && C > 0 && C % V == 0, "sde_act_bwd_bias: bad argument");
    SDE_CHECK_ARG(act == SDE_ACT_NONE || out, "sde_act_bwd_bias: activation backward needs the saved output");
    SDE_CHECK_ARG((dbias == nullptr) || (part && Cbias > 0 && Cbias <= C), "sde_act_bwd_bias: bias gradient needs a partial slab");
    hipStream_t s = (hipStream_t)stream;
    const int nblk = sde_reduce_num_blocks(M, C);
    const long rpb = (M + nblk - 1) / nblk;
    float* p = part;
    const size_t lds = ((size_t)C > 256 * 8 ? (size_t)C : 256 * 8) * sizeof(float);
    DISPATCH_T(dtype,
               hipLaunchKernelGGL(act_bwd_bias_kernel<float>, dim3(nblk), dim3(256), lds, s, (const float*)dout, (const float*)dout1, (const float*)out, act, M, C, rpb, (float*)dz, p),
               hipLaunchKernelGGL(act_bwd_bias_kernel<bf16_t>, dim3(nblk), dim3(256), lds, s, (const bf16_t*)dout, (const bf16_t*)dout1, (const bf16_t*)out, act, M, C, rpb, (bf16_t*)dz, p),
               hipLaunchKernelGGL(act_bwd_bias_kernel<half_t>, dim3(nblk), dim3(256), lds, s, (const half_t*)dout, (const half_t*)dout1, (const half_t*)out, act, M, C, rpb, (half_t*)dz, p));
    SDE_CHECK_LAUNCH("sde_act_bwd_bias");
    if (dbias) {
        int rows = nblk;
        const float* src = pre_reduce(part, rows, C, s);
        hipLaunchKernelGGL(colsum_finalize_kernel, dim3(sde_cdiv(Cbias, 16)), dim3(SLAB_T), 0, s, src, rows, C, Cbias, dbias, accumulate);
        SDE_CHECK_LAUNCH("sde_act_bwd_bias/finalize");
    }
    return SDE_OK;
}

int sde_colsum_finalize_batched(const sde_colsum_item* items, int n, sde_stream_t stream) {
    SDE_CHECK_ARG(items && n >= 0, "sde_colsum_finalize_batched: bad argument");
    for (int base = 0; base < n; base += COLSUM_MAX_ITEMS) {
        ColsumBatch b;
        b.n = n - base < COLSUM_MAX_ITEMS ? n - base : COLSUM_MAX_ITEMS;
        b.first[0] = 0;
        for (int k = 0; k < COLSUM_MAX_ITEMS; ++k) {
            const bool on = k < b.n;
            const sde_colsum_item* it = on ? items + base + k : nullptr;
            SDE_CHECK_ARG(!on || (it->part && it->out && it->rows >= 1 && it->rows <= 4096 && it->C >= 1 && it->C <= it->ld),
                          "sde_colsum_finalize_batched: item %d: bad slab (rows=%d ld=%d C=%d)", base + k, on ? it->rows : 0, on ? it->ld : 0, on ? it->C : 0);
            b.part[k] = on ? it->part : nullptr; b.out[k] = on ? it->out : nullptr;
            b.rows[k] = on ? it->rows : 0; b.ld[k] = on ? it->ld : 0; b.C[k] = on ? it->C : 0; b.accumulate[k] = on ? it->accumulate : 0;
            b.first[k + 1] = b.first[k] + (on ? sde_cdiv(it->C, 16) : 0);
        }
        if (b.first[b.n] == 0) continue;
        hipLaunchKernelGGL(colsum_finalize_batched_kernel, dim3(b.first[b.n]), dim3(SLAB_T), 0, (hipStream_t)stream, b);
        SDE_CHECK_LAUNCH("sde_colsum_finalize_batched");
    }
    return SDE_OK;
}

int sde_refl_fold(const void* dxp, int B, int H, int W, int C, int C0, int upcat, int dtype, void* dx0, void* dx1, sde_stream_t stream) {
    const int V = SDE_IS16(dtype) ? 8 : 4;
    SDE_CHECK_ARG(dxp && dx0 && B > 0 && H >= 2 && W >= 2 && C % V == 0, "sde_refl_fold: bad argument (B=%d H=%d W=%d C=%d)", B, H, W, C);
    SDE_CHECK_ARG(!upcat || (C0 > 0 && C0 <= C && C0 % V == 0 && H % 2 == 0 && W % 2 == 0 && (C0 == C || dx1)), "sde_refl_fold: bad upcat argument");
    hipStream_t s = (hipStream_t)stream;
    const long items = upcat ? (long)B * (H / 2) * (W / 2) * (C0 / V) + (long)B * H * W * ((C - C0) / V) : (long)B * H * W * (C / V);
    const int nb = grid_for(items);
    DISPATCH_T(dtype, hipLaunchKernelGGL(refl_fold_kernel<float>, dim3(nb), dim3(256), 0, s, (const float*)dxp, B, H, W, C, C0, upcat, (float*)dx0, (float*)dx1),
               hipLaunchKernelGGL(refl_fold_kernel<bf16_t>, dim3(nb), dim3(256), 0, s, (const bf16_t*)dxp, B, H, W, C, C0, upcat, (bf16_t*)dx0, (bf16_t*)dx1),
               hipLaunchKernelGGL(refl_fold_kernel<half_t>, dim3(nb), dim3(256), 0, s, (const half_t*)dxp, B, H, W, C, C0, upcat, (half_t*)dx0, (half_t*)dx1));
    SDE_CHECK_LAUNCH("sde_refl_fold");
    return SDE_OK;
}

int sde_depth_head_fwd(const void* y, int B, int H, int W, int ld, float min_depth, float max_depth, int flip, int dtype, float* depth, sde_stream_t stream) {
    SDE_CHECK_ARG(y && depth && B > 0 && H > 0 && W > 0 && ld > 0 && min_depth > 0 && max_depth > min_depth, "sde_depth_head_fwd: bad argument");
    hipStream_t s = (hipStream_t)stream;
    const float mind = 1.0f / max_depth, maxd = 1.0f / min_depth;
    const int nb = grid_for((long)B * H * W);
    DISPATCH_T(dtype, hipLaunchKernelGGL(depth_head_fwd_kernel<float>, dim3(nb), dim3(256), 0, s, (const float*)y, B, H, W, ld, mind, maxd, flip, depth),
               hipLaunchKernelGGL(depth_head_fwd_kernel<bf16_t>, dim3(nb), dim3(256), 0, s, (const bf16_t*)y, B, H, W, ld, mind, maxd, flip, depth),
               hipLaunchKernelGGL(depth_head_fwd_kernel<half_t>, dim3(nb), dim3(256), 0, s, (const half_t*)y, B, H, W, ld, mind, maxd, flip, depth));
    SDE_CHECK_LAUNCH("sde_depth_head_fwd");
    return SDE_OK;
}

int sde_depth_head_bwd(const void* y, const float* ddepth, int B, int H, int W, int ld, float min_depth, float max_depth, int flip, int dtype, void* dy,
                       sde_stream_t stream) {
    return sde_depth_head_bwd_bias(y, ddepth, B, H, W, ld, min_depth, max_depth, flip, dtype, dy, nullptr, nullptr, 0, stream);
}

int sde_depth_head_bias_blocks(int B, int H, int W) { return grid_for((long)B * H * W); }

int sde_depth_head_bwd_bias(const void* y, const float* ddepth, int B, int H, int W, int ld, float min_depth, float max_depth, int flip, int dtype, void* dy,
                            float* part, float* dbias, int accumulate, sde_stream_t stream) {
    SDE_CHECK_ARG(y && ddepth && dy && B > 0 && H > 0 && W > 0 && ld > 0, "sde_depth_head_bwd: bad argument");
    SDE_CHECK_ARG((part == nullptr) == (dbias == nullptr), "sde_depth_head_bwd_bias: the bias gradient needs both the partial buffer and the output");
    hipStream_t s = (hipStream_t)stream;
    const float mind = 1.0f / max_depth, maxd = 1.0f / min_depth;
    const int nb = grid_for((long)B * H * W);
    DISPATCH_T(dtype, hipLaunchKernelGGL(depth_head_bwd_kernel<float>, dim3(nb), dim3(256), 0, s, (const float*)y, ddepth, B, H, W, ld, mind, maxd, flip, (float*)dy, part),
               hipLaunchKernelGGL(depth_head_bwd_kernel<bf16_t>, dim3(nb), dim3(256), 0, s, (const bf16_t*)y, ddepth, B, H, W, ld, mind, maxd, flip, (bf16_t*)dy, part),
               hipLaunchKernelGGL(depth_head_bwd_kernel<half_t>, dim3(nb), dim3(256), 0, s, (const half_t*)y, ddepth, B, H, W, ld, mind, maxd, flip, (half_t*)dy, part));
    SDE_CHECK_LAUNCH("sde_depth_head_bwd");
    if (dbias) {
        hipLaunchKernelGGL(head_bias_finalize_kernel, dim3(1), dim3(256), 0, s, part, nb, dbias, accumulate);
        SDE_CHECK_LAUNCH("sde_depth_head_bwd_bias/finalize");
    }
    return SDE_OK;
}

int sde_gn_relu_fwd(const void* x, const float* gamma, const float* beta, int B, int HW, int C, int G, float eps, int relu, int dtype, float* part, float* gnp,
                    void* out, sde_stream_t stream) {
    return sde_gn_relu_res_fwd(x, nullptr, gamma, beta, B, HW, C, G, eps, relu, dtype, part, gnp, out, stream);
}

static bool gn_vector_path(int C, int dtype) { const int V = SDE_IS16(dtype) ? 8 : 4; return C % V == 0 && 256 % (C / V) == 0; }

int sde_gn_relu_res_fwd(const void* x, const void* res, const float* gamma, const float* beta, int B, int HW, int C, int G, float eps, int relu, int dtype,
                        float* part, float* gnp, void* out, sde_stream_t stream) {
    SDE_CHECK_ARG(x && gamma && beta && part && gnp && out && B > 0 && HW > 0 && C > 0 && G > 0 && C % G == 0, "sde_gn_relu_fwd: bad argument");
    SDE_CHECK_ARG(C % (SDE_IS16(dtype) ? 8 : 4) == 0, "sde_gn_relu_fwd: C=%d must be a multiple of the 16-byte group", C);
    SDE_CHECK_ARG(!res || gn_vector_path(C, dtype), "sde_gn_relu_res_fwd: the residual form needs C / (16-byte group) to divide 256 (C=%d)", C);
    hipStream_t s = (hipStream_t)stream;
    const size_t lds = 2 * (size_t)C * sizeof(float);
    DISPATCH_T(dtype, hipLaunchKernelGGL(gn_stats_kernel<float>, dim3(GN_CHUNKS, B), dim3(256), lds, s, (const float*)x, (const float*)res, HW, C, part),
               hipLaunchKernelGGL(gn_stats_kernel<bf16_t>, dim3(GN_CHUNKS, B), dim3(256), lds, s, (const bf16_t*)x, (const bf16_t*)res, HW, C, part),
               hipLaunchKernelGGL(gn_stats_kernel<half_t>, dim3(GN_CHUNKS, B), dim3(256), lds, s, (const half_t*)x, (const half_t*)res, HW, C, part));
    SDE_CHECK_LAUNCH("sde_gn_relu_fwd/stats");
    hipLaunchKernelGGL(gn_finalize_kernel, dim3(B * G), dim3(64), 0, s, part, B, C, G, HW, eps, gnp);
    SDE_CHECK_LAUNCH("sde_gn_relu_fwd/finalize");
    const int nb = grid_for((long)B * HW * (C / (SDE_IS16(dtype) ? 8 : 4)));
    DISPATCH_T(dtype, hipLaunchKernelGGL(gn_apply_kernel<float>, dim3(nb), dim3(256), 0, s, (const float*)x, (const float*)res, gnp, gamma, beta, B, HW, C, G, relu, (float*)out),
               hipLaunchKernelGGL(gn_apply_kernel<bf16_t>, dim3(nb), dim3(256), 0, s, (const bf16_t*)x, (const bf16_t*)res, gnp, gamma, beta, B, HW, C, G, relu, (bf16_t*)out),
               hipLaunchKernelGGL(gn_apply_kernel<half_t>, dim3(nb), dim3(256), 0, s, (const half_t*)x, (const half_t*)res, gnp, gamma, beta, B, HW, C, G, relu, (half_t*)out));
    SDE_CHECK_LAUNCH("sde_gn_relu_fwd/apply");
    return SDE_OK;
}

int sde_gn_relu_bwd(const void* dout, const void* out, const void* x, const float* gnp, const float* gamma, int B, int HW, int C, int G, int relu, int dtype,
                    float* part, float* coef, float* dgamma, float* dbeta, int accumulate_params, void* dx, sde_stream_t stream) {
    return sde_gn_relu_res_bwd(dout, out, x, nullptr, gnp, gamma, B, HW, C, G, relu, dtype, part, coef, dgamma, dbeta, accumulate_params, dx, stream);
}

int sde_gn_relu_res_bwd(const void* dout, const void* out, const void* x, const void* res, const float* gnp, const float* gamma, int B, int HW, int C, int G, int relu,
                        int dtype, float* part, float* coef, float* dgamma, float* dbeta, int accumulate_params, void* dx, sde_stream_t stream) {
    SDE_CHECK_ARG(dout && out && x && gnp && gamma && part && coef && dgamma && dbeta && dx && C % G == 0, "sde_gn_relu_bwd: bad argument");
    SDE_CHECK_ARG(!res || gn_vector_path(C, dtype), "sde_gn_relu_res_bwd: the residual form needs C / (16-byte group) to divide 256 (C=%d)", C);
    SDE_CHECK_ARG(C % (SDE_IS16(dtype) ? 8 : 4) == 0, "sde_gn_relu_bwd: C=%d must be a multiple of the 16-byte group", C);
    hipStream_t s = (hipStream_t)stream;
    const size_t lds = 2 * (size_t)C * sizeof(float);
    DISPATCH_T(dtype,
               hipLaunchKernelGGL(gn_bwd_stats_kernel<float>, dim3(GN_CHUNKS, B), dim3(256), lds, s, (const float*)dout, (const float*)out, (const float*)x, (const float*)res, gnp, HW, C, G, relu, part),
               hipLaunchKernelGGL(gn_bwd_stats_kernel<bf16_t>, dim3(GN_CHUNKS, B), dim3(256), lds, s, (const bf16_t*)dout, (const bf16_t*)out, (const bf16_t*)x, (const bf16_t*)res, gnp, HW, C, G, relu, part),
               hipLaunchKernelGGL(gn_bwd_stats_kernel<half_t>, dim3(GN_CHUNKS, B), dim3(256), lds, s, (const half_t*)dout, (const half_t*)out, (const half_t*)x, (const half_t*)res, gnp, HW, C, G, relu, part));
    SDE_CHECK_LAUNCH("sde_gn_relu_bwd/stats");
    hipLaunchKernelGGL(gn_bwd_finalize_kernel, dim3(B * G + C), dim3(64), 0, s, part, gamma, B, C, G, HW, coef, dgamma, dbeta, accumulate_params);
// ... 54 lines not shown
```

simpledepthestimation_amd/hip/nn.py:

```python
import contextlib
import ctypes
import functools
import os
import weakref
from collections import namedtuple
from ctypes import POINTER, Structure, c_float, c_int, c_int32, c_long, c_void_p

import torch

from . import lib as L

SRC_PLAIN, SRC_UPCAT, SRC_ZEROINS = 0, 1, 2
REDUCE_ROWS = 32
ACT_NONE, ACT_ELU, ACT_RELU = 0, 1, 2


class ConvDesc(Structure):
    _fields_ = [("x0", c_void_p), ("x1", c_void_p), ("dtype", c_int32), ("C0", c_int32), ("C1", c_int32), ("H0", c_int32), ("W0", c_int32),
                ("IH", c_int32), ("IW", c_int32), ("src_mode", c_int32), ("KH", c_int32), ("KW", c_int32), ("stride", c_int32), ("pad", c_int32),
                ("reflect", c_int32), ("Bn", c_int32), ("OH", c_int32), ("OW", c_int32)]


_P, _I, _F, _LG = c_void_p, c_int, c_float, c_long
L.register_protos({
    "sde_pack_weight": ([_P, _P, _I, _I, _I, _I, _I, _I, _I, _I, _P], c_int),
    "sde_pack_weights_batched": ([_P, _I, _LG, _I, _P], c_int),
    "sde_pack_item_blocks": ([_I, _I, _I, _I], c_int),
    "sde_conv_fwd": ([POINTER(ConvDesc), _P, _P, _I, _P, _I, _I, _P, _P], c_int),
    "sde_conv_fwd_tiles_m": ([POINTER(ConvDesc), _I], c_int),
    "sde_conv_fwd_ws_bytes": ([POINTER(ConvDesc), _I], ctypes.c_size_t),
    "sde_conv_fwd_ws": ([POINTER(ConvDesc), _P, _P, _I, _P, _I, _I, _P, _P, ctypes.c_size_t, _P], c_int),
    "sde_conv_fwd_variant": ([POINTER(ConvDesc), _I], c_int),
    "sde_conv_dgrad_bnbwd_rows": ([POINTER(ConvDesc), _I, _I], c_int),
    "sde_conv_dgrad_bnbwd": ([POINTER(ConvDesc), _P, _P, _I, _I, _P, _P, _P, _P], c_int),
    "sde_conv_dgrad_bnbwd_res_rows": ([POINTER(ConvDesc), _I, _I], c_int),
    "sde_conv_dgrad_bnbwd_res": ([POINTER(ConvDesc), _P, _P, _I, _I, _P, _P, _P, _P, _P, _P], c_int),
    "sde_bn_bwd_from_part": ([_P, _I, _P, _P, _P, _LG, _I, _I, _P, _P, _P, _I, _P, _P], c_int),
    "sde_conv_set_halo_min_blocks": ([_I], c_int),
    "sde_conv_set_option": ([_I, _I], c_int),
    "sde_kernel_lds_bytes": ([_I, _I], c_int),
    "sde_conv_wgrad_splits": ([POINTER(ConvDesc), _I], c_int),
    "sde_conv_wgrad_variant": ([POINTER(ConvDesc), _I, _I], c_int),
    "sde_conv_wgrad": ([POINTER(ConvDesc), _P, _I, _I, _I, _P, _I, _P, _I, _P], c_int),
    "sde_conv_wgrad_partial": ([POINTER(ConvDesc), _P, _I, _I, _P, _I, _P], c_int),
    "sde_wgrad_reduce_batched": ([_P, _I, _P], c_int),
    "sde_colsum_finalize_batched": ([_P, _I, _P], c_int),
    "sde_prep_input": ([_P, _P, _P, _I, _I, _I, _I, _I, _I, _I, _P, _P], c_int),
    "sde_bn_finalize": ([_P, _I, _I, _LG, _P, _P, _P, _P, _F, _F, _P, _P], c_int),
    "sde_bn_eval_params": ([_P, _P, _P, _P, _F, _I, _P, _P], c_int),
    "sde_bn_apply": ([_P, _P, _P, _I, _LG, _I, _I, _P, _P], c_int),
    "sde_bn_finalize_apply_ok": ([_I, _I, _I], c_int),
    "sde_bn_set_fuse": ([_I], c_int),
    "sde_bn_finalize_apply": ([_P, _I, _I, _LG, _P, _P, _P, _P, _F, _F, _P, _P, _P, _I, _I, _P, _P], c_int),
    "sde_reduce_num_blocks": ([_LG, _I], c_int),
    "sde_bn_bwd": ([_P, _P, _P, _P, _P, _P, _P, _I, _LG, _I, _I, _P, _P, _P, _P, _I, _P, _P, _P], c_int),
    "sde_maxpool_fwd": ([_P, _I, _I, _I, _I, _I, _P, _P, _P], c_int),
    "sde_depth_head_bias_blocks": ([_I, _I, _I], c_int),
    "sde_depth_head_bwd_bias": ([_P, _P, _I, _I, _I, _I, _F, _F, _I, _I, _P, _P, _P, _I, _P], c_int),
    "sde_maxpool_bwd": ([_P, _P, _I, _I, _I, _I, _I, _P, _P], c_int),
    "sde_maxpool_bwd_sum": ([_P, _P, _P, _I, _I, _I, _I, _I, _P, _P], c_int),
    "sde_act_bwd_bias": ([_P, _P, _I, _LG, _I, _I, _P, _P, _P, _I, _I, _P], c_int),
    "sde_act_bwd_bias_sum": ([_P, _P, _P, _I, _LG, _I, _I, _P, _P, _P, _I, _I, _P], c_int),
    "sde_refl_fold": ([_P, _I, _I, _I, _I, _I, _I, _I, _P, _P, _P], c_int),
    "sde_depth_head_fwd": ([_P, _I, _I, _I, _I, _F, _F, _I, _I, _P, _P], c_int),
    "sde_depth_head_bwd": ([_P, _P, _I, _I, _I, _I, _F, _F, _I, _I, _P, _P], c_int),
    "sde_gn_relu_fwd": ([_P, _P, _P, _I, _I, _I, _I, _F, _I, _I, _P, _P, _P, _P], c_int),
    "sde_gn_relu_bwd": ([_P, _P, _P, _P, _P, _I, _I, _I, _I, _I, _I, _P, _P, _P, _P, _I, _P, _P], c_int),
    "sde_gn_relu_res_fwd": ([_P, _P, _P, _P, _I, _I, _I, _I, _F, _I, _I, _P, _P, _P, _P], c_int),
    "sde_gn_relu_res_bwd": ([_P, _P, _P, _P, _P, _P, _I, _I, _I, _I, _I, _I, _P, _P, _P, _P, _I, _P, _P], c_int),
    "sde_space_to_depth": ([_P, _I, _I, _I, _I, _I, _P, _P], c_int),
    "sde_depth_to_space": ([_P, _I, _I, _I, _I, _I, _P, _P], c_int),
    "sde_concat_fwd": ([_P, _P, _P, _I, _I, _I, _I, _I, _I, _I, _I, _P, _P], c_int),
    "sde_concat_bwd": ([_P, _I, _I, _I, _I, _I, _I, _I, _I, _P, _P, _P, _P], c_int),
    "sde_inv_depth_head_fwd": ([_P, _I, _I, _I, _I, _F, _F, _F, _I, _I, _P, _P, _P], c_int),
    "sde_inv_depth_head_bwd": ([_P, _P, _P, _I, _I, _I, _I, _F, _F, _F, _I, _I, _P, _P], c_int),
    "sde_conv3d_fwd": ([_P, _P, _P, _I, _I, _I, _I, _I, _P, _P], c_int),
    "sde_conv3d_dgrad": ([_P, _P, _I, _I, _I, _I, _I, _P, _P], c_int),
    "sde_conv3d_wgrad_num_blocks": ([_I, _I, _I, _I, _I], c_int),
    "sde_conv3d_wgrad": ([_P, _P, _I, _I, _I, _I, _I, _P, _P, _P, _I, _P], c_int),
    "sde_adam_step": ([_P, _P, _P, _P, _LG, _P, _P], c_int),
    "sde_grad_check": ([_P, _LG, _P, _P], c_int),
    "sde_grad_norm": ([_P, _LG, _P, _P, _F, _F, _P], c_int),
    "sde_loss_scale_update": ([_P, _F, _F, _I, _P], c_int),
})


OPT_PGEMM, OPT_PGEMM_DEPTH, OPT_PGEMM_3X3, OPT_PGEMM_TILE, OPT_SPLITK, OPT_WGRAD_BLOCKS, OPT_WGRAD_HALO, OPT_CONV_SMALL, OPT_WGRAD_DMA, OPT_BNBWD_FUSE, OPT_CU_RESERVE = 1, 2, 3, 4, 5, 6, 7, 8, 9, 10, 11
OPT_WGRAD_DMA_RING, OPT_PGEMM_PER_CU = 12, 13
KERNEL_PGEMM, KERNEL_WGRAD_DMA, KERNEL_WGRAD_HALO, KERNEL_WGRAD_STAGED, KERNEL_WGRAD_SUM, KERNEL_WGRAD_REDUCE = 1, 2, 3, 4, 5, 6


def set_option(key, value):
    old = L.lib().sde_conv_set_option(int(key), int(value))
    if old < 0:
        raise L.SdeHipError(f"sde_conv_set_option({key}, {value}) failed: {L.lib().sde_last_error().decode()}")
    return old


def kernel_lds_bytes(kind, variant=0):
    n = L.lib().sde_kernel_lds_bytes(int(kind), int(variant))
    if n < 0:
        raise L.SdeHipError(f"sde_kernel_lds_bytes({kind}, {variant}): bad kind / variant")
    return n


WGRAD_HALO_KERNEL, WGRAD_DMA_KERNEL, WGRAD_STAGED_KERNEL = 1, 2, 3


def dtype_code(dt):
    if dt == torch.float32:
        return L.F32
    if dt == torch.bfloat16:
        return L.BF16
    if dt == torch.float16:
        return L.F16
    raise L.SdeHipError(f"unsupported activation dtype {dt}")


def vec_of(dt):
    return 4 if dt == torch.float32 else 8


def pad_to(c, v):
    return (c + v - 1) // v * v


def is_ohwi(t):
    return t.dim() == 4 and not t.is_contiguous() and t.permute(0, 2, 3, 1).is_contiguous()


def _dense(t):
    return t.is_contiguous() or is_ohwi(t)


def _grad_slot(p):
    g = p.grad if (p is not None and p.is_leaf) else None
    if g is not None and g.dtype == torch.float32 and _dense(g) and g.shape == p.shape:
        return g
    return None


def _f32(t):
    if t.dtype != torch.float32:
        raise L.SdeHipError("parameters must be float32")
    return t.contiguous()


def aliases(out, n):
    return out if n == 1 else (out,) + tuple(out.view(out.shape) for _ in range(n - 1))


def fan_in(douts, slots):
    grads = [g.contiguous() for g in douts if g is not None]
    if not grads:
        return ()
    for g in grads[slots:]:
        grads[slots - 1] = grads[slots - 1] + g
    return tuple(grads[:slots]) + (None,) * (slots - len(grads))


def pack_weight(w, dtype, cin_pad, cout_pad, for_dgrad=False):
    w = _f32(w)
    Cout, Cin, KH, KW = w.shape
    shape = (cin_pad, KH, KW, cout_pad) if for_dgrad else (cout_pad, KH, KW, cin_pad)
    out = torch.empty(shape, device=w.device, dtype=dtype)
    L.check(L.lib().sde_pack_weight(L.ptr(w), L.ptr(out), dtype_code(dtype), Cout, Cin, KH, KW, cin_pad, cout_pad, int(for_dgrad), L.stream()),
            "sde_pack_weight")
    return out


def _desc(x0, x1, src_mode, KH, KW, stride, pad, reflect, IH, IW, OH, OW):
    d = ConvDesc()
    B, H0, W0, C0 = x0.shape
    d.x0 = x0.data_ptr(); d.x1 = x1.data_ptr() if x1 is not None else 0
    d.dtype = dtype_code(x0.dtype)
    d.C0, d.C1, d.H0, d.W0, d.IH, d.IW = C0, (x1.shape[3] if x1 is not None else 0), H0, W0, IH, IW
    d.src_mode, d.KH, d.KW, d.stride, d.pad, d.reflect = src_mode, KH, KW, stride, pad, int(reflect)
    d.Bn, d.OH, d.OW = B, OH, OW
    return d


_timed = L.timed


def conv_raw(d, x_dtype, w_packed, bias, act, Cout, ldy, want_stats, device, kind="igemm_fwd", flops=0.0):
    y = torch.empty(d.Bn, d.OH, d.OW, ldy, device=device, dtype=x_dtype)
    stats, tiles = None, 0
    lib = L.lib()
    if want_stats:
        tiles = lib.sde_conv_fwd_tiles_m(ctypes.byref(d), ldy)
        stats = torch.empty(tiles + REDUCE_ROWS, Cout, 2, device=device, dtype=torch.float32)
    variant = lib.sde_conv_fwd_variant(ctypes.byref(d), ldy) if L.PROFILE is not None else 0
    meta = None
    if L.PROFILE is not None:
        esz = 4 if x_dtype == torch.float32 else 2
        meta = dict(M=d.Bn * d.OH * d.OW, N=ldy, K=d.KH * d.KW * (d.C0 + d.C1), k=d.KH, s=d.stride, mode=d.src_mode,
                    bytes=esz * (d.Bn * d.H0 * d.W0 * d.C0 + d.Bn * d.IH * d.IW * d.C1 + d.Bn * d.OH * d.OW * ldy))
    ws_bytes = lib.sde_conv_fwd_ws_bytes(ctypes.byref(d), ldy)
    ws = torch.empty(ws_bytes // 4, device=device, dtype=torch.float32) if ws_bytes else None
    _timed(kind, flops, variant, lambda: L.check(lib.sde_conv_fwd_ws(ctypes.byref(d), L.ptr(w_packed), L.ptr(bias), act, L.ptr(y), Cout, ldy, L.ptr(stats),
                                                                     L.ptr(ws), ws_bytes, L.stream()), "sde_conv_fwd_ws"), meta)
    return y, stats


class _Handovers:

    def __init__(self):
        self.bn_out = {}
        self.bn_out_res = {}
        self.bn_part = {}
        self.res_grad = {}
        self.head_slot = {}
        self.head_done = {}

    @staticmethod
    def _put(d, cap, t, ent):
        if len(d) > cap:
            d.clear()
        d[t.data_ptr()] = ent

    @staticmethod
    def _live(ent, t):
        return ent[1:] if (ent is not None and ent[0]() is t) else None

    def put_bn_out(self, out, y, bnp, res=False):
        (self.res_grad if res else self.bn_part).clear()
        self._put(self.bn_out_res if res else self.bn_out, 64, out, (weakref.ref(out), y, bnp))

    def take_bn_out(self, x, res=False):
        return self._live(self.bn_out_res.get(x.data_ptr()) if res else self.bn_out.pop(x.data_ptr(), None), x)

    def drop_bn_out_res(self, ptr):
        self.bn_out_res.pop(ptr, None)

    def put_bn_part(self, g, ent):
        self._put(self.bn_part, 16, g, ent)

    def take_bn_part(self, g, res=False):
        ent = self.bn_part.get(g.data_ptr())
        return self.bn_part.pop(g.data_ptr()) if (ent is not None and (not res or len(ent) == 4)) else None

    def put_res_grad(self, ptr, g, if_expected=False):
        if self.bn_out_res or not if_expected:
            self.res_grad[ptr] = g

    def take_res_grad(self, x):
        return self.res_grad.pop(x.data_ptr(), None)

    def put_head_slot(self, y, bias):
        self.head_done.clear()
        self._put(self.head_slot, 64, y, (weakref.ref(y), bias))

    def take_head_slot(self, y):
        return (self._live(self.head_slot.pop(y.data_ptr(), None), y) or (None,))[0]

    def put_head_done(self, dy, bias):
        self.head_done[dy.data_ptr()] = id(bias)

    def take_head_done(self, dy, bias):
        return self.head_done.pop(dy.data_ptr(), None) == id(bias)

    def drop_head_done(self, bias):
        n = len(self.head_done)
        self.head_done = {k: v for k, v in self.head_done.items() if v != id(bias)}
        return len(self.head_done) < n

    def end_phase(self):
        self.res_grad.clear()
        self.bn_part.clear()


_HANDOVER = _Handovers()


def _dgrad_bnbwd(dd, wd, dz, x0, Cv, bn, flops, res):
    lib = L.lib()
    g_other = _HANDOVER.take_res_grad(x0) if res else None
    if res and (g_other is None or not (g_other.shape == x0.shape and g_other.dtype == x0.dtype and g_other.is_contiguous())):
        return None
    name = "sde_conv_dgrad_bnbwd_res" if res else "sde_conv_dgrad_bnbwd"
    rows = getattr(lib, name + "_rows")(ctypes.byref(dd), Cv, Cv)
    if rows <= 0:
        if res:
            _HANDOVER.put_res_grad(x0.data_ptr(), g_other)
        return None
    y_bn, bnp = bn
    part = torch.empty(rows + REDUCE_ROWS, Cv, 2, device=x0.device, dtype=torch.float32)
    dx0 = torch.empty(x0.shape[:3] + (Cv,), device=x0.device, dtype=x0.dtype)
    variant = lib.sde_conv_fwd_variant(ctypes.byref(dd), Cv) if L.PROFILE is not None else 0
    meta = dict(M=dx0.numel() // Cv, N=Cv, K=dd.KH * dd.KW * dd.C0, k=dd.KH, s=1, mode=0,
                bytes=2 * (dz.numel() + (4 if res else 2) * dx0.numel())) if L.PROFILE is not None else None
    extra = (L.ptr(g_other), L.ptr(x0)) if res else ()
    _timed("igemm_dgrad", flops, variant, lambda: L.check(getattr(lib, name)(ctypes.byref(dd), L.ptr(wd), L.ptr(dx0), Cv, Cv, L.ptr(y_bn), L.ptr(bnp),
                                                                             L.ptr(part), *extra, L.stream()), name), meta)
    _HANDOVER.put_bn_part(dx0, (y_bn.data_ptr(), part, rows) + ((g_other.data_ptr(),) if res else ()))
    return dx0


class _Conv2d(torch.autograd.Function):
    @staticmethod
    def forward(ctx, x0, x1, weight, bias, stride, pad, reflect, act, upcat, want_stats, owner=None, n_out=1):
        ctx.set_materialize_grads(False)
        if n_out > 1 and want_stats:
            raise L.SdeHipError("conv2d: output aliases (n_out) belong to the BatchNorm that follows when statistics are requested")
        if not x0.is_contiguous() or (x1 is not None and not x1.is_contiguous()):
            raise L.SdeHipError("conv2d: NHWC inputs must be contiguous")
        dt = x0.dtype
        V = vec_of(dt)
        B, H0, W0, C0 = x0.shape
        Cout, Cin, KH, KW = weight.shape
        C1 = x1.shape[3] if x1 is not None else 0
        if C0 % V or C1 % V:
            raise L.SdeHipError(f"conv2d: channel counts ({C0},{C1}) must be multiples of {V}")
        if Cin > C0 + C1 or (upcat and Cin != C0 + C1):
            raise L.SdeHipError(f"conv2d: weight expects {Cin} input channels, tensors carry {C0}+{C1}")
        IH, IW = (2 * H0, 2 * W0) if upcat else (H0, W0)
        OH = (IH + 2 * pad - KH) // stride + 1
        OW = (IW + 2 * pad - KW) // stride + 1
        ldy = pad_to(Cout, V)
        d = _desc(x0, x1, SRC_UPCAT if upcat else SRC_PLAIN, KH, KW, stride, pad, reflect, IH, IW, OH, OW)
        pre = getattr(owner, "_packed", None) if owner is not None else None
        if pre is not None and pre[0].dtype == dt and pre[0].shape == (ldy, KH, KW, C0 + C1):
            wp, ctx.wd_pre = pre
        else:
            wp, ctx.wd_pre = pack_weight(weight, dt, C0 + C1, ldy), None
            if owner is not None:
                owner._pack_shapes = (dt, C0 + C1, ldy)
        b32 = _f32(bias) if bias is not None else None
        flops = 2.0 * B * OH * OW * Cout * KH * KW * Cin
        plain = x1 is None and not upcat and not reflect and stride == 1
        ent = _HANDOVER.take_bn_out(x0)
        ctx.bn_in = ent if plain else None
        ent = _HANDOVER.take_bn_out(x0, res=True) if RESBN_FUSED else None
        ctx.bn_in_res = ent if (plain and ctx.bn_in is None) else None
        y, stats = conv_raw(d, dt, wp, b32, act, Cout, ldy, want_stats, x0.device, "igemm_fwd", flops)
        ctx.save_for_backward(x0, x1, weight, y if act != ACT_NONE else None)
        ctx.params = (weight, bias)
        ctx.cfg = (stride, pad, reflect, act, upcat, bias is not None, IH, IW, OH, OW)
        ctx.want_stats = want_stats
        if HEAD_BIAS_FUSED and bias is not None and act == ACT_NONE and Cout == 1 and not want_stats and n_out == 1:
            _HANDOVER.put_head_slot(y, bias)
        if want_stats:
            ctx.mark_non_differentiable(stats)
            return y, stats
        return aliases(y, n_out)

    @staticmethod
    def backward(ctx, *douts):
        x0, x1, weight, y = ctx.saved_tensors
        dy, dy1 = fan_in(douts[:1] if ctx.want_stats else douts, 2) or (None, None)
        stride, pad, reflect, act, upcat, has_bias, IH, IW, OH, OW = ctx.cfg
        dt = x0.dtype
        V = vec_of(dt)
        lib = L.lib()
        dev = x0.device
        B, H0, W0, C0 = x0.shape
        C1 = x1.shape[3] if x1 is not None else 0
        Cout, Cin, KH, KW = weight.shape
        ldy = pad_to(Cout, V)
        if dy is None:
            return (None,) * 12
        off_main = MAIN_STREAM is not None and torch.cuda.current_stream() != MAIN_STREAM
        if off_main and not L.is_aux_stream(torch.cuda.current_stream()):
            raise L.SdeHipError("conv2d backward is running on a different stream than the one the backward phase started on; the "
                                "weight-gradient side-stream bookkeeping supports one main stream (plus the registered auxiliary stream) only")
        dy = dy.contiguous()
        M = B * OH * OW
        flops = 2.0 * M * Cout * KH * KW * Cin
        dbias = None
        dz = dy
        head_did_bias = has_bias and act == ACT_NONE and dy1 is None and _HANDOVER.take_head_done(dy, ctx.params[1])
        if has_bias and not head_did_bias and _HANDOVER.drop_head_done(ctx.params[1]):
            raise L.SdeHipError("conv2d backward: the one-channel output feeding depth_head has a second consumer; the fused disparity-head bias "
                                "gradient supports exactly one (set hip.nn.HEAD_BIAS_FUSED = False for such a graph)")
        if (act != ACT_NONE or has_bias or dy1 is not None) and not head_did_bias:
            nblk = lib.sde_reduce_num_blocks(M, ldy)
            part = torch.empty(nblk + REDUCE_ROWS, ldy, device=dev) if has_bias else None
            bslot = _grad_slot(ctx.params[1]) if has_bias else None
            dbias = (bslot if bslot is not None else torch.empty(Cout, device=dev)) if has_bias else None
            dz = torch.empty_like(dy) if (act != ACT_NONE or dy1 is not None) else None
            later = bslot is not None and WGRAD_DEFER.add_bias(part, nblk, ldy, Cout, bslot)
            L.check(lib.sde_act_bwd_bias_sum(L.ptr(dy), L.ptr(dy1), L.ptr(y), act, M, ldy, dtype_code(dt), L.ptr(dz), L.ptr(part), None if later else L.ptr(dbias), Cout,
                                             int(bslot is not None), L.stream()), "sde_act_bwd_bias_sum")
            if bslot is not None:
                dbias = None
            if dz is None:
                dz = dy
        need_dx = ctx.needs_input_grad[0] or (x1 is not None and ctx.needs_input_grad[1])
        dw = side = None
        if ctx.needs_input_grad[2]:
            d = _desc(x0, x1, SRC_UPCAT if upcat else SRC_PLAIN, KH, KW, stride, pad, reflect, IH, IW, OH, OW)
            splits = lib.sde_conv_wgrad_splits(ctypes.byref(d), Cout)
            wslot = _grad_slot(ctx.params[0])
            esz = 4 if dt == torch.float32 else 2
            meta = dict(M=M, N=Cout, K=KH * KW * (C0 + C1), k=KH, s=stride, mode=int(upcat), splits=splits,
                        bytes=esz * (B * H0 * W0 * C0 + B * IH * IW * C1 + M * ldy) + 8 * splits * Cout * KH * KW * (C0 + C1)) if L.PROFILE is not None else None
            dw = wslot if wslot is not None else torch.empty(weight.shape, device=dev)
            wflags = (1 if wslot is not None else 0) | (2 if is_ohwi(dw) else 0)
            op_bytes = (dz.numel() + x0.numel() + (x1.numel() if x1 is not None else 0)) * dz.element_size()
            dw, side = WGRAD_DEFER.weight_grad(WGradJob(d, dz, x0, x1, Cout, ldy, Cin, C0 + C1, KH * KW, splits, wslot, dw, wflags,
                                                        4 * splits * Cout * KH * KW * (C0 + C1), op_bytes, need_dx, off_main, flops, meta))
        dx0 = dx1 = None
        if need_dx:
            Cv = C0 + C1
            wd = ctx.wd_pre if ctx.wd_pre is not None else pack_weight(weight, dt, Cv, ldy, for_dgrad=True)
            if reflect:
                dd = _desc(dz, None, SRC_PLAIN, KH, KW, 1, KH - 1, False, OH, OW, IH + 2, IW + 2)
                dxp, _ = conv_raw(dd, dt, wd, None, ACT_NONE, Cv, Cv, False, dev, "igemm_dgrad", flops)
                dx0 = torch.empty_like(x0)
                dx1 = torch.empty_like(x1) if x1 is not None else None
                L.check(lib.sde_refl_fold(L.ptr(dxp), B, IH, IW, Cv, C0, int(upcat), dtype_code(dt), L.ptr(dx0), L.ptr(dx1), L.stream()), "sde_refl_fold")
            else:
                if upcat:
                    raise L.SdeHipError("upsample+concat source is only supported with reflection padding (decoder)")
                if stride == 1:
                    dd = _desc(dz, None, SRC_PLAIN, KH, KW, 1, KH - 1 - pad, False, OH, OW, IH, IW)
                    if ctx.bn_in_res is not None:
                        dx0 = _dgrad_bnbwd(dd, wd, dz, x0, Cv, ctx.bn_in_res, flops, res=True)
                    elif ctx.bn_in is not None and BNBWD_FUSED:
                        dx0 = _dgrad_bnbwd(dd, wd, dz, x0, Cv, ctx.bn_in, flops, res=False)
                elif stride == 2:
                    dd = _desc(dz, None, SRC_ZEROINS, KH, KW, 1, KH - 1 - pad, False, 2 * OH - 1, 2 * OW - 1, IH, IW)
# ... 37 lines not shown
    return False, "group", queued + 1 >= limit or queued_bytes + op_bytes >= budget_bytes


class WGradReducer:

    def __init__(self, defer=True):
        self.defer = defer
        self._drop()

    def _drop(self):
        self.first_group = None
        self.jobs, self._seen = [], set()
        self.bias_jobs, self._seen_bias = [], set()
        self.pending = []
        self.queue = []
        self.queue_bytes = 0
        self.groups_done = 0

    @contextlib.contextmanager
    def phase(self, device, phase_b=False):
        global WGRAD_DEFER, MAIN_STREAM
        WGRAD_DEFER, MAIN_STREAM = self, (torch.cuda.current_stream() if device.type == "cuda" else None)
        self.first_group = L.FIRST_GROUP_B if phase_b else None
        try:
            yield
            self.flush()
        finally:
            WGRAD_DEFER, MAIN_STREAM = _NO_PHASE, None
            _HANDOVER.end_phase()
            self.join_pending()
            self._drop()

    def weight_grad(self, j):
        fork = j.need_dx and L.SIDE_STREAM and L.PROFILE is None and not j.off_main
        if fork and L.FORK_MIN_BYTES:
            fork = j.op_bytes >= L.FORK_MIN_BYTES
        run_first, place, close = False, ("alone" if fork else "inline"), False
        if self.defer and not j.off_main:
            run_first, place, close = wgrad_group_rule(len(self.queue), self.queue_bytes, self.groups_done, j.op_bytes, j.need_dx, fork,
                                                       L.FIRST_GROUP if self.first_group is None else self.first_group,
                                                       L.WGRAD_GROUP, L.GROUP_MAX_BYTES, L.GROUP_BUDGET_BYTES, EARLY_TAIL)
        if run_first:
            self.run_queue()
        side = L.side_stream() if place != "inline" else None
        if place == "alone":
            self.join_pending(keep=L.JOIN_LAG - 1)
            side.wait_stream(torch.cuda.current_stream())
        ok = self.defer and j.wslot is not None and j.wslot.data_ptr() not in self._seen
        direct = (ok and j.splits == 1 and j.Cin_pad == j.Cin and (j.KHW == 1 or is_ohwi(j.wslot)) and j.wslot.data_ptr() % 16 == 0
                  and L.PROFILE is None)
        deferred = ok and not direct and j.slab_bytes <= L.DEFER_MAX_BYTES
        slab = j.wslot if direct else torch.empty(j.splits, j.Cout, j.KHW * j.Cin_pad, device=j.x0.device)
        if direct or deferred:
            self._seen.add(j.wslot.data_ptr())
        if deferred:
            self.jobs.append((slab, j.wslot, (slab.data_ptr(), j.wslot.data_ptr(), j.splits, j.Cout, j.KHW, j.Cin_pad, j.Cin, j.flags)))
        launch = functools.partial(self._launch, j, slab, "direct" if direct else "deferred" if deferred else "reduce", side)
        if place == "group":
            self.queue.append((launch, (j.dz, j.x0, j.x1, slab, j.dw)))
            self.queue_bytes += j.op_bytes
            if close:
                self.run_queue()
        else:
            with torch.cuda.stream(side) if side is not None else contextlib.nullcontext():
                launch()
        return (None if j.wslot is not None else j.dw), (side if place == "alone" else None)

    @staticmethod
    def _launch(j, slab, target, side):
        ring = L.wgrad_dma_ring() if side is not None else 0
        if ring:
            old = set_option(OPT_WGRAD_DMA_RING, ring)
            try:
                return WGradReducer._launch_ring(j, slab, target, side)
            finally:
                set_option(OPT_WGRAD_DMA_RING, old)
        return WGradReducer._launch_ring(j, slab, target, side)

    @staticmethod
    def _launch_ring(j, slab, target, side):
        lib = L.lib()
        if target == "reduce" and L.PROFILE is None:
            L.check(lib.sde_conv_wgrad(ctypes.byref(j.d), L.ptr(j.dz), j.Cout, j.ldy, j.Cin, L.ptr(slab), j.splits, _wptr(j.dw), j.flags, L.stream()),
                    "sde_conv_wgrad")
        else:
            rows = 1 if target == "direct" else j.splits
            _timed("wgrad", j.flops, 0, lambda: L.check(lib.sde_conv_wgrad_partial(ctypes.byref(j.d), L.ptr(j.dz), j.Cout, j.ldy, _wptr(slab), rows,
                                                                                   L.stream()), "sde_conv_wgrad_partial"), j.meta)
            if target == "reduce":
                one = (WReduceItem * 1)(WReduceItem(slab.data_ptr(), j.dw.data_ptr(), j.splits, j.Cout, j.KHW, j.Cin_pad, j.Cin, j.flags))
                _timed("wgrad_reduce", 0.0, 0, lambda: L.check(lib.sde_wgrad_reduce_batched(one, 1, L.stream()), "sde_wgrad_reduce_batched"),
                       dict(jobs=1))
        if side is not None and target != "direct":
            slab.record_stream(side)

    def join(self, side, operands):
        if side is not None and L.JOIN_LAG > 0 and self.defer:
            self.pending.append((side.record_event(), operands))
        elif side is not None:
            torch.cuda.current_stream().wait_stream(side)

    def run_queue(self):
        if not self.queue:
            return
        side = L.side_stream()
        self.join_pending(keep=L.JOIN_LAG - 1)
        side.wait_stream(torch.cuda.current_stream())
        with torch.cuda.stream(side):
            for launch, _ in self.queue:
                launch()
        self.pending.append((side.record_event(), [operands for _, operands in self.queue]))
        self.queue, self.queue_bytes = [], 0
        self.groups_done += 1

    def join_pending(self, keep=0):
        while len(self.pending) > max(0, keep):
            torch.cuda.current_stream().wait_event(self.pending.pop(0)[0])

    def add_bias(self, part, rows, ld, C, bslot):
        if not (self.defer and BIAS_DEFER and L.PROFILE is None and bslot.data_ptr() not in self._seen_bias):
            return False
        self._seen_bias.add(bslot.data_ptr())
        self.bias_jobs.append((part, rows, ld, C, bslot))
        return True

    def flush(self):
        self.run_queue()
        self.groups_done = 0
        self.join_pending()
        if self.bias_jobs:
            arr = (ColsumItem * len(self.bias_jobs))(*[ColsumItem(p.data_ptr(), b.data_ptr(), r, ld, C, 1) for p, r, ld, C, b in self.bias_jobs])
            L.check(L.lib().sde_colsum_finalize_batched(arr, len(self.bias_jobs), L.stream()), "sde_colsum_finalize_batched")
        self.bias_jobs, self._seen_bias = [], set()
        if not self.jobs:
            return
        items = []
        for slab, wslot, it in self.jobs:
            src, dwp, rows, Cout, KHW, Cin_pad, Cin_real, _ = it
            lo, hi = slab.data_ptr(), slab.data_ptr() + slab.numel() * 4
            if not (src is not None and lo <= src and src + rows * Cout * KHW * Cin_pad * 4 <= hi and wslot.numel() == Cout * Cin_real * KHW
                    and dwp == wslot.data_ptr() and Cin_real <= Cin_pad and rows >= 1):
                raise L.SdeHipError(f"WGradReducer: inconsistent job (slab {tuple(slab.shape)}, src offset {None if src is None else src - lo}, "
                                    f"rows {rows}, Cout {Cout}, KHW {KHW}, Cin_pad {Cin_pad}, Cin_real {Cin_real}, slot {tuple(wslot.shape)})")
            items.append(WReduceItem(*it))
        arr = (WReduceItem * len(items))(*items)
        _timed("wgrad_reduce", 0.0, 0, lambda: L.check(L.lib().sde_wgrad_reduce_batched(arr, len(items), L.stream()), "sde_wgrad_reduce_batched"),
               dict(jobs=len(items)))
        self.jobs, self._seen = [], set()


FUSE_BN_FINALIZE = True
BNBWD_FUSED = True
BNBWD_HITS = 0
RESBN_FUSED = os.environ.get("SDE_RESBN", "1") != "0"
RESBN_HITS = 0
_NO_PHASE = WGradReducer(defer=False)
WGRAD_DEFER = _NO_PHASE
MAIN_STREAM = None
FOLD_ROWS = 16


class PackItem(Structure):
    _fields_ = [("src", c_void_p), ("dst_fwd", c_void_p), ("dst_dgrad", c_void_p), ("Cout", c_int32), ("Cin", c_int32), ("KH", c_int32), ("KW", c_int32),
                ("Cin_pad", c_int32), ("Cout_pad", c_int32), ("src_layout", c_int32), ("reserved", c_int32), ("end", ctypes.c_int64)]


class WeightPacker:

    def __init__(self, model):
        import numpy as np
        convs = [m for m in model.modules() if getattr(m, "_pack_shapes", None) is not None]
        if not convs:
            raise L.SdeHipError("WeightPacker: run one forward pass first")
        self.dtype = convs[0]._pack_shapes[0]
        items, end = [], 0
        self._keep = []
        for m in convs:
            dt, cin_pad, ldy = m._pack_shapes
            if dt != self.dtype:
                raise L.SdeHipError("WeightPacker: mixed compute dtypes")
            w = m.weight
            Cout, Cin, KH, KW = w.shape
            wp = torch.empty(ldy, KH, KW, cin_pad, device=w.device, dtype=dt)
            wd = torch.empty(cin_pad, KH, KW, ldy, device=w.device, dtype=dt)
            m._packed = (wp, wd)
            nb = L.lib().sde_pack_item_blocks(ldy, cin_pad, KH, KW)
            if nb <= 0:
                raise L.SdeHipError(f"WeightPacker: unsupported kernel size {KH}x{KW}")
            end += nb
            if not _dense(w):
                raise L.SdeHipError("WeightPacker: conv weights must be dense (OIHW or channels-last)")
            items.append((w.data_ptr(), wp.data_ptr(), wd.data_ptr(), Cout, Cin, KH, KW, cin_pad, ldy, 1 if is_ohwi(w) else 0, 0, end))
            self._keep.append((w, wp, wd))
        dev = convs[0].weight.device

        def table(rows):
            arr = (PackItem * len(rows))(*[PackItem(*it) for it in rows])
            return torch.from_numpy(np.frombuffer(bytes(arr), dtype=np.uint8).copy()).to(dev)
        self.items = table(items)
        self.n, self.total = len(items), end
        self._ptrs = [w.data_ptr() for w, _, _ in self._keep]

    def run(self):
        if any(w.data_ptr() != p for (w, _, _), p in zip(self._keep, self._ptrs)):
            raise L.SdeHipError("WeightPacker: a weight tensor moved (e.g. flattened after the packer was built); rebuild the packer")
        L.check(L.lib().sde_pack_weights_batched(L.ptr(self.items), self.n, self.total, dtype_code(self.dtype), L.stream()), "sde_pack_weights_batched")


def conv2d(x, weight, bias=None, stride=1, pad=0, reflect=False, act=ACT_NONE, skip=None, upsample=False, bn_stats=False, owner=None, n_out=1):
    return _Conv2d.apply(x, skip, weight, bias, int(stride), int(pad), bool(reflect), int(act), bool(upsample), bool(bn_stats), owner, int(n_out))


DECONV_DIRECT = True
DECONV_RULE = True


def deconv_direct(B, H, W, C, ldy, esize):
    if not DECONV_DIRECT:
        return False
    if not DECONV_RULE:
        return True
    workgroups = B * ((H + 7) // 8) * ((W + 15) // 16) * ((ldy + 31) // 32 if ldy > 16 else 1)
    return not (C * esize >= 16 * 64 and workgroups < 256)


class _ConvTranspose2d(torch.autograd.Function):

    @staticmethod
    def forward(ctx, x, weight, bias, act, owner=None):
        if not x.is_contiguous():
            raise L.SdeHipError("conv_transpose2d: the NHWC input must be contiguous")
        if act not in (ACT_NONE, ACT_RELU):
            raise L.SdeHipError(f"conv_transpose2d: activation {act} is not supported (ACT_NONE, ACT_RELU)")
        dt = x.dtype
        if dt not in (torch.float32, torch.bfloat16):
            raise L.SdeHipError(f"conv_transpose2d runs in fp32 or bf16, not {dt}")
        V = vec_of(dt)
        B, H, W, C = x.shape
        Cin, Cout, KH, KW = weight.shape
        if (KH, KW) != (3, 3):
            raise L.SdeHipError("conv_transpose2d: 3x3 kernels only")
        if C % V or Cin > C:
            raise L.SdeHipError(f"conv_transpose2d: weight expects {Cin} input channels, the tensor carries {C} (multiples of {V})")
        ldy = pad_to(Cout, V)
        pre = getattr(owner, "_packed", None) if owner is not None else None
        if pre is not None and pre[0].dtype == dt and pre[0].shape == (C, 3, 3, ldy):
            ctx.wb_pre, wf = pre
        else:
            wf, ctx.wb_pre = pack_weight(weight, dt, ldy, C, for_dgrad=True), None
            if owner is not None:
                owner._pack_shapes = (dt, ldy, C)
        b32 = _f32(bias) if bias is not None else None
        flops = 2.0 * B * H * W * 9 * Cin * Cout
        lib = L.lib()
        if deconv_direct(B, H, W, C, ldy, x.element_size()):
            y = torch.empty(B, 2 * H, 2 * W, ldy, device=x.device, dtype=dt)
            meta = dict(M=4 * B * H * W, N=ldy, K=9 * C // 4, k=3, s=2, mode=3, bytes=x.element_size() * (x.numel() + y.numel())) if L.PROFILE is not None else None
            _timed("igemm_fwd", flops, 0, lambda: L.check(lib.sde_deconv3x3s2_fwd(L.ptr(x), L.ptr(wf), L.ptr(b32), act, B, H, W, C, Cout, ldy, dtype_code(dt),
                                                                                   L.ptr(y), L.stream()), "sde_deconv3x3s2_fwd"), meta)
        else:
            d = _desc(x, None, SRC_ZEROINS, 3, 3, 1, 1, False, 2 * H - 1, 2 * W - 1, 2 * H, 2 * W)
            y, _ = conv_raw(d, dt, wf, b32, ACT_NONE, Cout, ldy, False, x.device, "igemm_fwd", flops)
            if act == ACT_RELU:
                z, y = y, torch.empty_like(y)
                L.check(lib.sde_relu_fwd(L.ptr(z), z.numel(), dtype_code(dt), L.ptr(y), L.stream()), "sde_relu_fwd")
        ctx.save_for_backward(x, weight, y if act != ACT_NONE else None)
        ctx.params = (weight, bias)
        ctx.act = act
        return y

    @staticmethod
    def backward(ctx, dy):
        x, weight, y = ctx.saved_tensors
        act, has_bias = ctx.act, ctx.params[1] is not None
        dt = x.dtype
        V = vec_of(dt)
        lib = L.lib()
        dev = x.device
        B, H, W, C = x.shape
        Cin, Cout = weight.shape[:2]
        ldy = pad_to(Cout, V)
        off_main = MAIN_STREAM is not None and torch.cuda.current_stream() != MAIN_STREAM
        if off_main and not L.is_aux_stream(torch.cuda.current_stream()):
            raise L.SdeHipError("conv_transpose2d backward is running on a different stream than the one the backward phase started on")
        dy = dy.contiguous()
        M = B * 4 * H * W
        flops = 2.0 * B * H * W * 9 * Cin * Cout
        dbias, dz = None, dy
        if act != ACT_NONE or has_bias:
            nblk = lib.sde_reduce_num_blocks(M, ldy)
            part = torch.empty(nblk + REDUCE_ROWS, ldy, device=dev) if has_bias else None
            bslot = _grad_slot(ctx.params[1]) if has_bias else None
            dbias = (bslot if bslot is not None else torch.empty(Cout, device=dev)) if has_bias else None
            dz = torch.empty_like(dy) if act != ACT_NONE else None
            later = bslot is not None and WGRAD_DEFER.add_bias(part, nblk, ldy, Cout, bslot)
            L.check(lib.sde_act_bwd_bias_sum(L.ptr(dy), None, L.ptr(y), act, M, ldy, dtype_code(dt), L.ptr(dz), L.ptr(part), None if later else L.ptr(dbias), Cout,
                                             int(bslot is not None), L.stream()), "sde_act_bwd_bias_sum")
            if bslot is not None:
                dbias = None
            if dz is None:
                dz = dy
        need_dx = ctx.needs_input_grad[0]
        d = _desc(dz, None, SRC_PLAIN, 3, 3, 2, 1, False, 2 * H, 2 * W, H, W)
        dw = side = None
        if ctx.needs_input_grad[1]:
            splits = lib.sde_conv_wgrad_splits(ctypes.byref(d), Cin)
# ... 11 lines not shown
            wb = ctx.wb_pre if ctx.wb_pre is not None else pack_weight(weight, dt, ldy, C)
            dx, _ = conv_raw(d, dt, wb, None, ACT_NONE, Cin, C, False, dev, "igemm_dgrad", flops)
        WGRAD_DEFER.join(side, (dz, x))
        return dx, dw, dbias, None, None


def conv_transpose2d(x, weight, bias=None, act=ACT_NONE, owner=None):
    return _ConvTranspose2d.apply(x, weight, bias, int(act), owner)


GCONV_DIRECT = True
GCONV_CG = (4, 8, 16, 32, 64)


def _gconv_check(x, weight, groups, stride):
    if x.dim() != 4 or weight.dim() != 4:
        raise L.SdeHipError("grouped_conv3x3: x is NHWC [B,H,W,C], weight [C, C/groups, 3, 3]")
    if x.dtype not in (torch.float32, torch.bfloat16):
        raise L.SdeHipError(f"grouped_conv3x3 runs in fp32 or bf16, not {x.dtype}")
    C, Cg, KH, KW = weight.shape
    if (KH, KW) != (3, 3):
        raise L.SdeHipError(f"grouped_conv3x3: 3x3 kernels only, got {KH}x{KW}")
    if stride not in (1, 2):
        raise L.SdeHipError(f"grouped_conv3x3: stride 1 or 2 only, got {stride}")
    if groups <= 0 or C != Cg * groups or x.shape[3] != C:
        raise L.SdeHipError(f"grouped_conv3x3: channel mismatch: the weight {tuple(weight.shape)} with {groups} groups maps {Cg * groups} -> {C} channels, "
                            f"the tensor carries {x.shape[3]} (input and output channels must be equal)")
    if Cg not in GCONV_CG or C % 16:
        raise L.SdeHipError(f"grouped_conv3x3: {Cg} channels per group of {C} are not supported: channels per group in {GCONV_CG}, channels a multiple of 16")
    if weight.dtype != torch.float32 or not _dense(weight):
        raise L.SdeHipError("grouped_conv3x3: the weight must be a dense float32 tensor (OIHW or channels-last)")
    if not x.is_contiguous():
        raise L.SdeHipError("grouped_conv3x3: the NHWC input must be contiguous")


class _GroupedConv3x3(torch.autograd.Function):

    @staticmethod
    def forward(ctx, x, weight, groups, stride, want_stats, n_out):
        ctx.set_materialize_grads(False)
        if n_out > 1 and want_stats:
            raise L.SdeHipError("grouped_conv3x3: output aliases (n_out) belong to the BatchNorm that follows when statistics are requested")
        _HANDOVER.take_bn_out(x)
        B, H, W, C = x.shape
        Cg = C // groups
        OH, OW = (H - 1) // stride + 1, (W - 1) // stride + 1
        lib, code = L.lib(), dtype_code(x.dtype)
        y = torch.empty(B, OH, OW, C, device=x.device, dtype=x.dtype)
        stats = None
        if want_stats:
            rows = lib.sde_gconv3x3_stats_rows(B, H, W, C, groups, stride, code)
            if rows <= 0:
                raise L.SdeHipError(f"sde_gconv3x3_stats_rows failed: {lib.sde_last_error().decode()}")
            stats = torch.empty(rows + REDUCE_ROWS, C, 2, device=x.device, dtype=torch.float32)
        flops = 2.0 * B * OH * OW * C * 9 * Cg
        meta = dict(M=B * OH * OW, N=C, K=9 * Cg, k=3, s=stride, mode=4, bytes=x.element_size() * (x.numel() + y.numel())) if L.PROFILE is not None else None
        _timed("igemm_fwd", flops, 0, lambda: L.check(lib.sde_gconv3x3_fwd(L.ptr(x), _wptr(weight), int(is_ohwi(weight)), B, H, W, C, groups, stride, code, L.ptr(y),
                                                                           L.ptr(stats), L.stream()), "sde_gconv3x3_fwd"), meta)
        ctx.save_for_backward(x, weight)
        ctx.param = weight
        ctx.cfg = (groups, stride, want_stats)
        if want_stats:
            ctx.mark_non_differentiable(stats)
            return y, stats
        return aliases(y, n_out)

    @staticmethod
    def backward(ctx, *douts):
        x, weight = ctx.saved_tensors
        groups, stride, want_stats = ctx.cfg
        grads = fan_in(douts[:1] if want_stats else douts, 1)
        if not grads:
            return (None,) * 6
        dz = grads[0]
        B, H, W, C = x.shape
        Cg = C // groups
        M = B * dz.shape[1] * dz.shape[2]
        lib, code = L.lib(), dtype_code(x.dtype)
        flops = 2.0 * M * C * 9 * Cg
        esz = x.element_size()
        dx = dw = None
        if ctx.needs_input_grad[0]:
            dx = torch.empty_like(x)
            meta = dict(M=B * H * W, N=C, K=9 * Cg, k=3, s=stride, mode=4, bytes=esz * (dz.numel() + dx.numel())) if L.PROFILE is not None else None
            _timed("igemm_dgrad", flops, 0, lambda: L.check(lib.sde_gconv3x3_dgrad(L.ptr(dz), _wptr(weight), int(is_ohwi(weight)), B, H, W, C, groups, stride, code,
                                                                                   L.ptr(dx), L.stream()), "sde_gconv3x3_dgrad"), meta)
        if ctx.needs_input_grad[1]:
            wslot = _grad_slot(ctx.param)
            dw = wslot if wslot is not None else torch.empty(weight.shape, device=x.device)
            wflags = (1 if wslot is not None else 0) | (2 if is_ohwi(dw) else 0)
            ws_bytes = lib.sde_gconv3x3_wgrad_ws_bytes(B, H, W, C, groups, stride, code)
            ws = torch.empty(ws_bytes // 4, device=x.device, dtype=torch.float32)
            meta = dict(M=M, N=C, K=9 * Cg, k=3, s=stride, mode=4, bytes=esz * (dz.numel() + x.numel()) + 2 * ws_bytes) if L.PROFILE is not None else None
            def call():
                L.check(lib.sde_gconv3x3_wgrad(L.ptr(x), L.ptr(dz), B, H, W, C, groups, stride, code, L.ptr(ws), ws_bytes, _wptr(dw), wflags, L.stream()), "sde_gconv3x3_wgrad")
            if wslot is None or L.PROFILE_REPEAT == 1:
                _timed("wgrad", flops, 0, call, meta)
            else:
                call()
            if wslot is not None:
                dw = None
        return dx, dw, None, None, None, None


def _gconv_dense_weight(weight, groups):
    C, Cg = weight.shape[:2]
    co = torch.arange(C, device=weight.device)
    ci = (co // Cg * Cg)[:, None] + torch.arange(Cg, device=weight.device)[None, :]
    return torch.zeros(C, C, 3, 3, device=weight.device, dtype=weight.dtype).index_put((co[:, None], ci), weight)


def grouped_conv3x3(x, weight, groups, stride=1, bn_stats=False, n_out=1):
    groups, stride = int(groups), int(stride)
    _gconv_check(x, weight, groups, stride)
    if GCONV_DIRECT:
        return _GroupedConv3x3.apply(x, weight, groups, stride, bool(bn_stats), int(n_out))
    return conv2d(x, _gconv_dense_weight(weight, groups), None, stride, 1, bn_stats=bn_stats, n_out=n_out)


class _BatchNormAct(torch.autograd.Function):

    @staticmethod
    def forward(ctx, y, stats, gamma, beta, running_mean, running_var, residual, relu, momentum, eps, training, n_out):
        ctx.set_materialize_grads(False)
        dt = y.dtype
        C = y.shape[-1]
        M = y.numel() // C
        lib = L.lib()
        dev = y.device
        bnp = torch.empty(4, C, device=dev)
        out = torch.empty_like(y)
        tiles = stats.shape[0] - REDUCE_ROWS if training else 0
        if training and FUSE_BN_FINALIZE and lib.sde_bn_finalize_apply_ok(tiles, C, dtype_code(dt)):
            L.check(lib.sde_bn_finalize_apply(L.ptr(stats), tiles, C, M, L.ptr(_f32(gamma)), L.ptr(_f32(beta)), L.ptr(running_mean), L.ptr(running_var),
                                              momentum, eps, L.ptr(bnp), L.ptr(y), L.ptr(residual), int(relu), dtype_code(dt), L.ptr(out), L.stream()),
                    "sde_bn_finalize_apply")
        else:
            if training:
                L.check(lib.sde_bn_finalize(L.ptr(stats), tiles, C, M, L.ptr(_f32(gamma)), L.ptr(_f32(beta)), L.ptr(running_mean), L.ptr(running_var),
                                            momentum, eps, L.ptr(bnp), L.stream()), "sde_bn_finalize")
            else:
                L.check(lib.sde_bn_eval_params(L.ptr(_f32(gamma)), L.ptr(_f32(beta)), L.ptr(running_mean), L.ptr(running_var), eps, C, L.ptr(bnp), L.stream()),
                        "sde_bn_eval_params")
            L.check(lib.sde_bn_apply(L.ptr(y), L.ptr(bnp), L.ptr(residual), int(relu), M, C, dtype_code(dt), L.ptr(out), L.stream()), "sde_bn_apply")
        ctx.save_for_backward(y, out if (relu and residual is not None) else None, bnp, gamma)
        ctx.params = (gamma, beta)
        ctx.cfg = (relu, residual is not None, training)
        if training and relu and residual is None and n_out == 1 and dt != torch.float32 and C % 64 == 0 and ctx.needs_input_grad[0] and BNBWD_FUSED:
            _HANDOVER.put_bn_out(out, y, bnp)
        ctx.res_ptr = residual.data_ptr() if residual is not None else None
        if training and relu and residual is not None and n_out == 2 and dt != torch.float32 and C % 64 == 0 and ctx.needs_input_grad[0] and BNBWD_FUSED and RESBN_FUSED:
            _HANDOVER.put_bn_out(out, y, bnp, res=True)
            ctx.res_tag = out.data_ptr()
        return aliases(out, n_out)

    @staticmethod
    def backward(ctx, *douts):
        y, out, bnp, gamma = ctx.saved_tensors
        relu, has_res, training = ctx.cfg
        if getattr(ctx, "res_tag", None) is not None:
            _HANDOVER.drop_bn_out_res(ctx.res_tag)
        if not training:
            raise L.SdeHipError("BatchNorm backward in eval mode is not on the path")
        grads = [d for d in fan_in(douts, 3) if d is not None]
        if not grads:
            return (None,) * 12
        dt = y.dtype
        C = y.shape[-1]
        M = y.numel() // C
        lib = L.lib()
        dev = y.device
        coef = torch.empty(2, C, device=dev)
        gs, bs = _grad_slot(ctx.params[0]), _grad_slot(ctx.params[1])
        direct = gs is not None and bs is not None
        dgamma = gs if direct else torch.empty(C, device=dev)
        dbeta = bs if direct else torch.empty(C, device=dev)
        dy = torch.empty_like(y)
        ent = _HANDOVER.take_bn_part(grads[0], res=has_res) if (relu and len(grads) == 1 + has_res) else None
        fits = ent is not None and ent[0] == y.data_ptr() and grads[0].shape == y.shape and grads[0].dtype == dt
        if has_res and ent is not None and not (fits and ent[3] == grads[1].data_ptr()):
            raise L.SdeHipError("BatchNorm backward: a data gradient that already contains the skip path's gradient arrived at a BatchNorm it was not "
                                "formed for (hip.nn.RESBN_FUSED = False selects the separate reduce pass)")
        if fits:
            global BNBWD_HITS, RESBN_HITS
            RESBN_HITS += has_res
            BNBWD_HITS += not has_res
            gm = grads[0]
            L.check(lib.sde_bn_bwd_from_part(L.ptr(ent[1]), ent[2], L.ptr(gm), L.ptr(y), L.ptr(bnp), M, C, dtype_code(dt), L.ptr(coef), L.ptr(dgamma),
                                             L.ptr(dbeta), int(direct), L.ptr(dy), L.stream()), "sde_bn_bwd_from_part")
            if has_res and ctx.res_ptr is not None:
                _HANDOVER.put_res_grad(ctx.res_ptr, gm)
            if direct:
                dgamma = dbeta = None
            return dy, None, dgamma, dbeta, None, None, (gm if has_res else None), None, None, None, None, None
        part = torch.empty(lib.sde_reduce_num_blocks(M, C) + REDUCE_ROWS, C, 2, device=dev)
        gm = torch.empty_like(y) if (relu or len(grads) > 1) else None
        d0, d1, d2 = (grads + [None, None])[:3]
        L.check(lib.sde_bn_bwd(L.ptr(d0), L.ptr(d1), L.ptr(d2), L.ptr(out), L.ptr(y), L.ptr(bnp), L.ptr(gamma), int(relu), M, C, dtype_code(dt), L.ptr(part),
                               L.ptr(coef), L.ptr(dgamma), L.ptr(dbeta), int(direct), L.ptr(gm), L.ptr(dy), L.stream()), "sde_bn_bwd")
        dres = (gm if gm is not None else d0) if has_res else None
        if dres is not None and ctx.res_ptr is not None and RESBN_FUSED:
            _HANDOVER.put_res_grad(ctx.res_ptr, dres, if_expected=True)
        if direct:
            dgamma = dbeta = None
        return dy, None, dgamma, dbeta, None, None, dres, None, None, None, None, None


def batch_norm_act(y, stats, gamma, beta, running_mean, running_var, residual=None, relu=True, momentum=0.1, eps=1e-5, training=True, n_out=1):
    return _BatchNormAct.apply(y, stats, gamma, beta, running_mean, running_var, residual, bool(relu), float(momentum), float(eps), bool(training), int(n_out))


class _MaxPool(torch.autograd.Function):
    @staticmethod
    def forward(ctx, x, n_out=1):
        ctx.set_materialize_grads(False)
        B, H, W, C = x.shape
        OH, OW = (H - 1) // 2 + 1, (W - 1) // 2 + 1
        out = torch.empty(B, OH, OW, C, device=x.device, dtype=x.dtype)
        idx = torch.empty(B, OH, OW, C, device=x.device, dtype=torch.uint8)
        L.check(L.lib().sde_maxpool_fwd(L.ptr(x.contiguous()), B, H, W, C, dtype_code(x.dtype), L.ptr(out), L.ptr(idx), L.stream()), "sde_maxpool_fwd")
        ctx.save_for_backward(idx)
        ctx.shape = (B, H, W, C)
        return aliases(out, n_out)

    @staticmethod
    def backward(ctx, *douts):
        (idx,) = ctx.saved_tensors
        B, H, W, C = ctx.shape
        grads = fan_in(douts, 2)
        if not grads:
            return None, None
        d0, d1 = grads
        dx = torch.empty(B, H, W, C, device=d0.device, dtype=d0.dtype)
        L.check(L.lib().sde_maxpool_bwd_sum(L.ptr(d0), L.ptr(d1), L.ptr(idx), B, H, W, C, dtype_code(d0.dtype), L.ptr(dx), L.stream()), "sde_maxpool_bwd_sum")
        return dx, None


def max_pool_3x3_s2(x, n_out=1):
    return _MaxPool.apply(x, int(n_out))


def prep_input(img, mean, std, dtype, flip=False):
    if img.dtype != torch.float32:
        raise L.SdeHipError("prep_input expects a float32 NCHW image")
    img = img.contiguous()
    B, C, H, W = img.shape
    Cp = pad_to(C, vec_of(dtype))
    out = torch.empty(B, H, W, Cp, device=img.device, dtype=dtype)
    m = _f32(mean.reshape(-1)) if mean is not None else None
    s = _f32(std.reshape(-1)) if std is not None else None
    L.check(L.lib().sde_prep_input(L.ptr(img), L.ptr(m), L.ptr(s), B, C, H, W, Cp, int(bool(flip)), dtype_code(dtype), L.ptr(out), L.stream()), "sde_prep_input")
    return out


HEAD_BIAS_HITS = 0
HEAD_BIAS_FUSED = True


class _DepthHead(torch.autograd.Function):
    @staticmethod
    def forward(ctx, y, min_depth, max_depth, flip):
        ctx.bias_param = _HANDOVER.take_head_slot(y)
        B, H, W, ld = y.shape
        depth = torch.empty(B, 1, H, W, device=y.device, dtype=torch.float32)
        L.check(L.lib().sde_depth_head_fwd(L.ptr(y.contiguous()), B, H, W, ld, min_depth, max_depth, int(flip), dtype_code(y.dtype), L.ptr(depth), L.stream()),
                "sde_depth_head_fwd")
        ctx.save_for_backward(y)
        ctx.cfg = (min_depth, max_depth, flip)
        return depth

    @staticmethod
    def backward(ctx, ddepth):
        (y,) = ctx.saved_tensors
        min_depth, max_depth, flip = ctx.cfg
        B, H, W, ld = y.shape
        dy = torch.empty_like(y)
        lib = L.lib()
        bslot = _grad_slot(ctx.bias_param) if ctx.bias_param is not None else None
        if bslot is not None and bslot.numel() == 1:
            part = torch.empty(lib.sde_depth_head_bias_blocks(B, H, W), device=y.device)
            L.check(lib.sde_depth_head_bwd_bias(L.ptr(y), L.ptr(ddepth.contiguous().float()), B, H, W, ld, min_depth, max_depth, int(flip), dtype_code(y.dtype),
                                                L.ptr(dy), L.ptr(part), L.ptr(bslot), 1, L.stream()), "sde_depth_head_bwd_bias")
            global HEAD_BIAS_HITS
            HEAD_BIAS_HITS += 1
            _HANDOVER.put_head_done(dy, ctx.bias_param)
        else:
            L.check(lib.sde_depth_head_bwd(L.ptr(y), L.ptr(ddepth.contiguous().float()), B, H, W, ld, min_depth, max_depth, int(flip), dtype_code(y.dtype),
                                           L.ptr(dy), L.stream()), "sde_depth_head_bwd")
        return dy, None, None, None


def depth_head(y, min_depth, max_depth, flip=False):
    return _DepthHead.apply(y, float(min_depth), float(max_depth), bool(flip))


class _GroupNormReLU(torch.autograd.Function):
    @staticmethod
    def forward(ctx, x, gamma, beta, groups, eps, relu, res=None):
        B, H, W, C = x.shape
        dev = x.device
        part = torch.empty(B, GN_CHUNKS, C, 2, device=dev)
        gnp = torch.empty(B, groups, 2, device=dev)
        out = torch.empty_like(x)
        x = x.contiguous()
        if res is not None:
            if res.shape != x.shape or res.dtype != x.dtype:
                raise L.SdeHipError("group_norm_relu: the residual must have the input's shape and dtype")
            res = res.contiguous()
        L.check(L.lib().sde_gn_relu_res_fwd(L.ptr(x), L.ptr(res), L.ptr(_f32(gamma)), L.ptr(_f32(beta)), B, H * W, C, groups, eps, int(relu), dtype_code(x.dtype),
                                            L.ptr(part), L.ptr(gnp), L.ptr(out), L.stream()), "sde_gn_relu_res_fwd")
        ctx.save_for_backward(x, out, gnp, gamma, res)
        ctx.params = (gamma, beta)
        ctx.cfg = (groups, relu)
        return out

    @staticmethod
    def backward(ctx, dout):
        x, out, gnp, gamma, res = ctx.saved_tensors
        groups, relu = ctx.cfg
        B, H, W, C = x.shape
        dev = x.device
        part = torch.empty(B, GN_CHUNKS, C, 2, device=dev)
        coef = torch.empty(B, groups, 2, device=dev)
        gs, bs = _grad_slot(ctx.params[0]), _grad_slot(ctx.params[1])
        direct = gs is not None and bs is not None
        dgamma = gs if direct else torch.empty(C, device=dev)
        dbeta = bs if direct else torch.empty(C, device=dev)
        dx = torch.empty_like(x)
        L.check(L.lib().sde_gn_relu_res_bwd(L.ptr(dout.contiguous()), L.ptr(out), L.ptr(x), L.ptr(res), L.ptr(gnp), L.ptr(_f32(gamma)), B, H * W, C, groups, int(relu),
                                            dtype_code(x.dtype), L.ptr(part), L.ptr(coef), L.ptr(dgamma), L.ptr(dbeta), int(direct), L.ptr(dx), L.stream()),
                "sde_gn_relu_res_bwd")
        if direct:
            dgamma = dbeta = None
        return dx, dgamma, dbeta, None, None, None, (dx if res is not None else None)


GN_CHUNKS = 64
GN_ACT = {False: 0, True: 1, "none": 0, "relu": 1, "elu": 2}


def group_norm_relu(x, gamma, beta, groups=16, eps=1e-5, relu=True, residual=None):
    if x.shape[-1] != gamma.numel():
        raise L.SdeHipError("group_norm_relu: channel padding is not supported (PoseNet / PackNet channels are multiples of 16)")
    return _GroupNormReLU.apply(x, gamma, beta, int(groups), float(eps), GN_ACT[relu], residual)


def _s2d(x, inverse):
    x = x.contiguous()
    B, H, W, C = x.shape
    if inverse:
        y = torch.empty(B, 2 * H, 2 * W, C // 4, device=x.device, dtype=x.dtype)
        L.check(L.lib().sde_depth_to_space(L.ptr(x), B, H, W, C, dtype_code(x.dtype), L.ptr(y), L.stream()), "sde_depth_to_space")
    else:
        y = torch.empty(B, H // 2, W // 2, 4 * C, device=x.device, dtype=x.dtype)
        L.check(L.lib().sde_space_to_depth(L.ptr(x), B, H, W, C, dtype_code(x.dtype), L.ptr(y), L.stream()), "sde_space_to_depth")
    return y


class _SpaceToDepth(torch.autograd.Function):
    @staticmethod
    def forward(ctx, x, inverse):
        ctx.inverse = inverse
        return _s2d(x, inverse)

    @staticmethod
    def backward(ctx, dy):
        return _s2d(dy, not ctx.inverse), None


def space_to_depth(x):
    return _SpaceToDepth.apply(x, False)


def depth_to_space(x):
    return _SpaceToDepth.apply(x, True)


class _Concat(torch.autograd.Function):
    @staticmethod
    def forward(ctx, p0, p1, inv, add):
        p0 = p0.contiguous()
        B, H, W, C0 = p0.shape
        V = vec_of(p0.dtype)
        C1 = p1.shape[3] if p1 is not None else 0
        if p1 is not None:
            p1 = p1.contiguous()
# ... 147 lines not shown
```

Baseline: 1931 images/s.

## Fuse max-pool backward into the preceding BatchNorm-ReLU backward reduction

The stem max-pool's backward no longer writes its own dx. It hands the pooled gradients and index map over to the BatchNorm+ReLU backward, which gathers the pool gradient inline while doing its reduction. This removes a full-resolution write and reread of the stem gradient tensor. The change also rewrites the standalone max-pool backward with 32-bit index math and a capped grid, and adds a vectorized input-prep kernel for padded channel counts. In exchange it brings a Python-side handover protocol that raises errors if the gradient reaches an unexpected consumer, plus extra gather work inside the reduction loop.

```diff
diff --git a/include/sde_hip.h b/include/sde_hip.h
--- a/include/sde_hip.h
+++ b/include/sde_hip.h
@@ -198,6 +198,9 @@
 int sde_bn_bwd(const void* dout, const void* dout1, const void* dout2, const void* out, const void* y, const float* bnp, const float* gamma, int relu,
                long M, int C, int dtype, float* part, float* coef, float* dgamma, float* dbeta, int accumulate_params, void* gm, void* dy,
                sde_stream_t stream);
+int sde_bn_bwd_pooled(const void* pool_d0, const void* pool_d1, const uint8_t* pool_idx, int B, int H, int W, const void* dout1, const void* dout2,
+                      const void* out, const void* y, const float* bnp, int relu, int C, int dtype, float* part, float* coef, float* dgamma, float* dbeta,
+                      int accumulate_params, void* gm, void* dy, sde_stream_t stream);
 int sde_bn_bwd_from_part(const float* part, int rows, const void* gm, const void* y, const float* bnp, long M, int C, int dtype, float* coef,
                          float* dgamma, float* dbeta, int accumulate_params, void* dy, sde_stream_t stream);
 
diff --git a/simpledepthestimation_amd/csrc/nn.hip b/simpledepthestimation_amd/csrc/nn.hip
--- a/simpledepthestimation_amd/csrc/nn.hip
+++ b/simpledepthestimation_amd/csrc/nn.hip
@@ -9,13 +9,11 @@
 template <> struct VecOf<bf16_t> { static constexpr int V = 8; };
 template <> struct VecOf<half_t> { static constexpr int V = 8; };
 
-template <typename T> __device__ __forceinline__ void load_vec(const T* p, float* v);
-template <> __device__ __forceinline__ void load_vec<float>(const float* p, float* v) {
-    const float4 t = *reinterpret_cast<const float4*>(p);
-    v[0] = t.x; v[1] = t.y; v[2] = t.z; v[3] = t.w;
-}
-template <> __device__ __forceinline__ void load_vec<bf16_t>(const bf16_t* p, float* v) {
-    const uint4 t = *reinterpret_cast<const uint4*>(p);
+template <typename T> __device__ __forceinline__ void unpack_vec(const uint4& t, float* v);
+template <> __device__ __forceinline__ void unpack_vec<float>(const uint4& t, float* v) {
+    v[0] = __uint_as_float(t.x); v[1] = __uint_as_float(t.y); v[2] = __uint_as_float(t.z); v[3] = __uint_as_float(t.w);
+}
+template <> __device__ __forceinline__ void unpack_vec<bf16_t>(const uint4& t, float* v) {
     const uint32_t w[4] = {t.x, t.y, t.z, t.w};
 #pragma unroll
     for (int i = 0; i < 4; ++i) {
@@ -23,12 +21,13 @@
         v[2 * i + 1] = __uint_as_float(w[i] & 0xffff0000u);
     }
 }
-template <> __device__ __forceinline__ void load_vec<half_t>(const half_t* p, float* v) {
+template <> __device__ __forceinline__ void unpack_vec<half_t>(const uint4& t, float* v) {
     typedef __attribute__((ext_vector_type(8))) _Float16 h8;
-    const h8 t = *reinterpret_cast<const h8*>(p);
-#pragma unroll
-    for (int i = 0; i < 8; ++i) v[i] = (float)t[i];
-}
+    const h8 h = __builtin_bit_cast(h8, t);
+#pragma unroll
+    for (int i = 0; i < 8; ++i) v[i] = (float)h[i];
+}
+template <typename T> __device__ __forceinline__ void load_vec(const T* p, float* v) { unpack_vec<T>(*reinterpret_cast<const uint4*>(p), v); }
 template <typename T> __device__ __forceinline__ void store_vec(T* p, const float* v);
 template <> __device__ __forceinline__ void store_vec<float>(float* p, const float* v) {
     *reinterpret_cast<float4*>(p) = make_float4(v[0], v[1], v[2], v[3]);
@@ -64,6 +63,36 @@
             }
             o[c] = (T)v;
         }
+    }
+}
+
+template <typename T, typename I>
+__global__ void __launch_bounds__(256) prep_input_vec_kernel(const float* __restrict__ img, const float* __restrict__ mean, const float* __restrict__ std_,
+                                                             int B, int C, int H, int W, int flip, T* __restrict__ out) {
+    constexpr int CP = VecOf<T>::V;
+    float m[CP], sd[CP];
+#pragma unroll
+    for (int c = 0; c < CP; ++c) {
+        m[c] = (mean && c < C) ? mean[c] : 0.f;
+        sd[c] = (mean && c < C) ? std_[c] : 1.f;
+    }
+    const I n = (I)B * H * W;
+    const long plane = (long)H * W;
+    for (I i = (I)blockIdx.x * 256 + threadIdx.x; i < n; i += (I)gridDim.x * 256) {
+        const I row = i / (I)W;
+        const int x = (int)(i - row * (I)W), b = (int)(row / (I)H), y = (int)(row - (I)b * (I)H);
+        const float* p = img + ((long)b * C * H + y) * W + (flip ? W - 1 - x : x);
+        float v[CP];
+#pragma unroll
+        for (int c = 0; c < CP; ++c) {
+            float t = 0.f;
+            if (c < C) {
+                t = p[c * plane];
+                if (mean) t = (t - m[c]) / sd[c];
+            }
+            v[c] = t;
+        }
+        store_vec<T>(out + (long)i * CP, v);
     }
 }
 
@@ -279,9 +308,73 @@
 }
 
 template <typename T, int V>
+__device__ __forceinline__ void pool_grad(const T* __restrict__ d0, const T* __restrict__ d1, const uint8_t* __restrict__ idx, int b, int ih, int iw, int OH,
+                                          int OW, int cch, int col, float* g) {
+    const int oh[2] = {(ih + 1) >> 1, (ih - 1) >> 1}, ow[2] = {(iw + 1) >> 1, (iw - 1) >> 1};
+    const int kh[2] = {(ih & 1) ? 0 : 1, 2}, kw[2] = {(iw & 1) ? 0 : 1, 2};
+    const bool vh[2] = {oh[0] < OH, (ih & 1) != 0}, vw[2] = {ow[0] < OW, (iw & 1) != 0};
+    uint4 r0[4], r1[4];
+    uint32_t ib[4][2];
+    uint32_t code[4];
+#pragma unroll
+    for (int n = 0; n < 4; ++n) {
+        const int a = n >> 1, c = n & 1;
+        r0[n] = make_uint4(0u, 0u, 0u, 0u); r1[n] = r0[n];
+        ib[n][0] = ib[n][1] = 0u;
+        code[n] = 255u;
+        if (vh[a] && vw[c]) {
+            const long o = ((((long)b * OH + oh[a]) * OW + ow[c]) * cch + col) * V;
+            r0[n] = *reinterpret_cast<const uint4*>(d0 + o);
+            if (d1) r1[n] = *reinterpret_cast<const uint4*>(d1 + o);
+            if (V == 8) {
+                const uint2 t = *reinterpret_cast<const uint2*>(idx + o);
+                ib[n][0] = t.x; ib[n][1] = t.y;
+            } else {
+                ib[n][0] = *reinterpret_cast<const uint32_t*>(idx + o);
+            }
+            code[n] = (uint32_t)(kh[a] * 3 + kw[c]);
+        }
+    }
+#pragma unroll
+    for (int e = 0; e < V; ++e) g[e] = 0.f;
+#pragma unroll
+    for (int n = 0; n < 4; ++n) {
+        if (code[n] == 255u) continue;
+        float d[V];
+        unpack_vec<T>(r0[n], d);
+        if (d1) {
+            float t[V];
+            unpack_vec<T>(r1[n], t);
+#pragma unroll
+            for (int e = 0; e < V; ++e) d[e] += t[e];
+        }
+#pragma unroll
+        for (int e = 0; e < V; ++e) g[e] += ((ib[n][e >> 2] >> (8 * (e & 3))) & 0xffu) == code[n] ? d[e] : 0.f;
+    }
+}
+
+struct PoolSrc {
+    const void* d1;
+    const uint8_t* idx;
+    int H, W, OH, OW;
+};
+
+struct PoolPos { int b, ih, iw, col; };
+
+__device__ __forceinline__ PoolPos pool_pos_of(unsigned item, int cch, const PoolSrc& ps) {
+    const unsigned pix = item / (unsigned)cch, row = pix / (unsigned)ps.W, b = row / (unsigned)ps.H;
+    return PoolPos{(int)b, (int)(row - b * (unsigned)ps.H), (int)(pix - row * (unsigned)ps.W), (int)(item - pix * (unsigned)cch)};
+}
+
+template <typename T, int V, bool POOL = false>
 __device__ __forceinline__ void bn_load_dz(const T* d0, const T* d1, const T* d2, const T* out, int relu, long off, float* d, const float* yv,
-                                           const float* sc, const float* sf) {
-    load_vec<T>(d0 + off, d);
+                                           const float* sc, const float* sf, int cch = 0, const PoolSrc* ps = nullptr, const PoolPos* pp = nullptr) {
+    if (POOL) {
+        pool_grad<T, V>(d0, (const T*)ps->d1, ps->idx, pp->b, pp->ih, pp->iw, ps->OH, ps->OW, cch, pp->col, d);
+        round_vec<T, V>(d);
+    } else {
+        load_vec<T>(d0 + off, d);
+    }
     if (d1) {
         float t[V];
         load_vec<T>(d1 + off, t);
@@ -305,11 +398,11 @@
     }
 }
 
-template <typename T, int NT = 256>
+template <typename T, int NT = 256, bool POOL = false>
 __global__ void __launch_bounds__(NT) bn_bwd_reduce_kernel(const T* __restrict__ dout, const T* __restrict__ dout1, const T* __restrict__ dout2,
                                                            const T* __restrict__ out, const T* __restrict__ y,
                                                            const float* __restrict__ bnp, int relu, long M, int C, long rows_per_block,
-                                                           float* __restrict__ part, T* __restrict__ gm) {
+                                                           float* __restrict__ part, T* __restrict__ gm, const PoolSrc ps) {
     constexpr int V = VecOf<T>::V;
     extern __shared__ float sh[];
     const int cch = C / V;
@@ -321,11 +414,25 @@
             mean[e] = bnp[c0 + e]; rstd[e] = bnp[C + c0 + e]; sc[e] = bnp[2 * C + c0 + e]; sf[e] = bnp[3 * C + c0 + e];
             acc[e] = 0.f; acc[V + e] = 0.f;
         }
-        const long total = M * cch;
-        for (long i = (long)blockIdx.x * NT + threadIdx.x; i < total; i += (long)gridDim.x * NT) {
+        const long total = M * cch, stride = (long)gridDim.x * NT;
+        PoolPos pp = {0, 0, 0, col}, dp = pp;
+        if (POOL) {
+            pp = pool_pos_of((unsigned)((long)blockIdx.x * NT + threadIdx.x), cch, ps);
+            dp = pool_pos_of((unsigned)stride, cch, ps);
+        }
+        for (long i = (long)blockIdx.x * NT + threadIdx.x; i < total; i += stride) {
             float d[V], yv[V];
             load_vec<T>(y + i * V, yv);
-            bn_load_dz<T, V>(dout, dout1, dout2, out, relu, i * V, d, yv, sc, sf);
+            bn_load_dz<T, V, POOL>(dout, dout1, dout2, out, relu, i * V, d, yv, sc, sf, cch, &ps, &pp);
+            if (POOL) {
+                pp.iw += dp.iw;
+                const int cw = pp.iw >= ps.W;
+                pp.iw -= cw ? ps.W : 0;
+                pp.ih += dp.ih + cw;
+                const int ch = pp.ih >= ps.H;
+                pp.ih -= ch ? ps.H : 0;
+                pp.b += dp.b + ch;
+            }
             if (gm) {
                 round_vec<T, V>(d);
                 store_vec<T>(gm + i * V, d);
@@ -352,7 +459,9 @@
         const long off = (r0 * cch + i) * V;
         float d[V], yv[V];
         load_vec<T>(y + off, yv);
-        bn_load_dz<T, V>(dout, dout1, dout2, out, relu, off, d, yv, bnp + 2 * C + c0, bnp + 3 * C + c0);
+        PoolPos pp = {0, 0, 0, col};
+        if (POOL) pp = pool_pos_of((unsigned)(off / V), cch, ps);
+        bn_load_dz<T, V, POOL>(dout, dout1, dout2, out, relu, off, d, yv, bnp + 2 * C + c0, bnp + 3 * C + c0, cch, &ps, &pp);
         if (gm) {
             round_vec<T, V>(d);
             store_vec<T>(gm + off, d);
@@ -502,47 +611,18 @@
     }
 }
 
-template <typename T>
+template <typename T, typename I>
 __global__ void __launch_bounds__(256) maxpool_bwd_kernel(const T* __restrict__ dout, const T* __restrict__ dout1, const uint8_t* __restrict__ idx, int B, int H,
                                                           int W, int C, int OH, int OW, T* __restrict__ dx) {
     constexpr int V = VecOf<T>::V;
     const int cch = C / V;
-    const long total = (long)B * H * W * cch;
-    for (long i = (long)blockIdx.x * 256 + threadIdx.x; i < total; i += (long)gridDim.x * 256) {
-        const int col = (int)(i % cch);
-        const long pix = i / cch;
-        const int iw = (int)(pix % W), ih = (int)((pix / W) % H), b = (int)(pix / ((long)W * H));
+    const I total = (I)B * H * W * cch;
+    for (I i = (I)blockIdx.x * 256 + threadIdx.x; i < total; i += (I)gridDim.x * 256) {
+        const I pix = i / (I)cch, row = pix / (I)W;
+        const int col = (int)(i - pix * (I)cch), iw = (int)(pix - row * (I)W), b = (int)(row / (I)H), ih = (int)(row - (I)b * (I)H);
         float g[V];
-#pragma unroll
-        for (int e = 0; e < V; ++e) g[e] = 0.f;
-#pragma unroll
-        for (int kh = 0; kh < 3; ++kh) {
-            const int t = ih + 1 - kh;
-            if (t < 0 || (t & 1)) continue;
-            const int oh = t >> 1;
-            if (oh >= OH) continue;
-#pragma unroll
-            for (int kw = 0; kw < 3; ++kw) {
-                const int u = iw + 1 - kw;
-                if (u < 0 || (u & 1)) continue;
-                const int ow = u >> 1;
-                if (ow >= OW) continue;
-                const long o = ((((long)b * OH + oh) * OW + ow) * cch + col) * V;
-                float d[V];
-                load_vec<T>(dout + o, d);
-                if (dout1) {
-                    float t[V];
-                    load_vec<T>(dout1 + o, t);
-#pragma unroll
-                    for (int e = 0; e < V; ++e) d[e] += t[e];
-                }
-                const uint8_t* ip = idx + o;
-#pragma unroll
-                for (int e = 0; e < V; ++e)
-                    if (ip[e] == kh * 3 + kw) g[e] += d[e];
-            }
-        }
-        store_vec<T>(dx + i * V, g);
+        pool_grad<T, V>(dout, dout1, idx, b, ih, iw, OH, OW, cch, col, g);
+        store_vec<T>(dx + (long)i * V, g);
     }
 }
 
@@ -1216,6 +1296,14 @@
     SDE_CHECK_ARG((mean == nullptr) == (std_ == nullptr), "sde_prep_input: mean/std must both be given or both be null");
     hipStream_t s = (hipStream_t)stream;
     const int nb = grid_for((long)B * H * W);
+    if (Cpad == (SDE_IS16(dtype) ? 8 : 4)) {
+#define SDE_PREP_VEC(T, I) hipLaunchKernelGGL((prep_input_vec_kernel<T, I>), dim3(nb), dim3(256), 0, s, img, mean, std_, B, C, H, W, flip, (T*)out)
+        if ((long)B * H * W < (1L << 31)) DISPATCH_T(dtype, SDE_PREP_VEC(float, unsigned), SDE_PREP_VEC(bf16_t, unsigned), SDE_PREP_VEC(half_t, unsigned));
+        else DISPATCH_T(dtype, SDE_PREP_VEC(float, long), SDE_PREP_VEC(bf16_t, long), SDE_PREP_VEC(half_t, long));
+#undef SDE_PREP_VEC
+        SDE_CHECK_LAUNCH("sde_prep_input");
+        return SDE_OK;
+    }
     DISPATCH_T(dtype, hipLaunchKernelGGL(prep_input_kernel<float>, dim3(nb), dim3(256), 0, s, img, mean, std_, B, C, H, W, Cpad, flip, (float*)out),
                hipLaunchKernelGGL(prep_input_kernel<bf16_t>, dim3(nb), dim3(256), 0, s, img, mean, std_, B, C, H, W, Cpad, flip, (bf16_t*)out),
                hipLaunchKernelGGL(prep_input_kernel<half_t>, dim3(nb), dim3(256), 0, s, img, mean, std_, B, C, H, W, Cpad, flip, (half_t*)out));
@@ -1297,34 +1385,44 @@
     return (int)nb;
 }
 
-int sde_bn_bwd(const void* dout, const void* dout1, const void* dout2, const void* out, const void* y, const float* bnp, const float* gamma, int relu,
-               long M, int C, int dtype, float* part, float* coef, float* dgamma, float* dbeta, int accumulate_params, void* gm, void* dy,
-               sde_stream_t stream) {
+}
+
+namespace {
+
+template <typename T, int NT, bool POOL>
+void launch_bn_reduce(int nblk, size_t lds, hipStream_t s, const void* dout, const void* dout1, const void* dout2, const void* out, const void* y, const float* bnp,
+                      int relu, long M, int C, long rpb, float* part, void* gm, const PoolSrc& ps) {
+    hipLaunchKernelGGL((bn_bwd_reduce_kernel<T, NT, POOL>), dim3(nblk), dim3(NT), lds, s, (const T*)dout, (const T*)dout1, (const T*)dout2, (const T*)out,
+                       (const T*)y, bnp, relu, M, C, rpb, part, (T*)gm, ps);
+}
+
+int bn_bwd_impl(const char* who, const void* dout, const void* dout1, const void* dout2, const void* out, const void* y, const float* bnp, int relu, long M, int C,
+                int dtype, float* part, float* coef, float* dgamma, float* dbeta, int accumulate_params, void* gm, void* dy, const PoolSrc* pool,
+                sde_stream_t stream) {
     const int V = SDE_IS16(dtype) ? 8 : 4;
-    SDE_CHECK_ARG(dout && y && bnp && part && coef && dgamma && dbeta && dy && M > 0 && C > 0 && C % V == 0, "sde_bn_bwd: bad argument");
+    SDE_CHECK_ARG(dout && y && bnp && part && coef && dgamma && dbeta && dy && M > 0 && C > 0 && C % V == 0, "%s: bad argument", who);
     if (relu && !out) relu = 2;
-    SDE_CHECK_ARG(gm || (!relu && !dout1 && !dout2), "sde_bn_bwd: a masked or summed gradient needs the gm buffer");
-    SDE_CHECK_ARG(dout1 || !dout2, "sde_bn_bwd: dout2 without dout1");
-    (void)gamma;
+    SDE_CHECK_ARG(gm || (!relu && !dout1 && !dout2 && !pool), "%s: a masked, summed or pooled gradient needs the gm buffer", who);
+    SDE_CHECK_ARG(dout1 || !dout2, "%s: dout2 without dout1", who);
     hipStream_t s = (hipStream_t)stream;
     int nblk = sde_reduce_num_blocks(M, C);
     const long rpb = (M + nblk - 1) / nblk;
     const size_t lds = (2 * (size_t)C > 256 * 16 ? 2 * (size_t)C : 256 * 16) * sizeof(float);
     const int cch = C / V;
     const bool wide = g_bn_fuse && g_bn_wide && SDE_IS16(dtype) && C % 64 == 0 && nblk > BNFA_MAX_ROWS && cch <= 256 && 256 % cch == 0;
+    const PoolSrc ps = pool ? *pool : PoolSrc{nullptr, nullptr, 0, 0, 0, 0};
+#define SDE_BN_REDUCE(T, NT, LDS)                                                                                                           \
+    do {                                                                                                                                    \
+        if (pool) launch_bn_reduce<T, NT, true>(nblk, LDS, s, dout, dout1, dout2, out, y, bnp, relu, M, C, rpb, part, gm, ps);               \
+        else launch_bn_reduce<T, NT, false>(nblk, LDS, s, dout, dout1, dout2, out, y, bnp, relu, M, C, rpb, part, gm, ps);                   \
+    } while (0)
     if (wide) {
         nblk = (nblk + 3) / 4;
-        if (dtype == SDE_BF16)
-            hipLaunchKernelGGL((bn_bwd_reduce_kernel<bf16_t, 1024>), dim3(nblk), dim3(1024), 1024 * 16 * sizeof(float), s, (const bf16_t*)dout, (const bf16_t*)dout1,
-                               (const bf16_t*)dout2, (const bf16_t*)out, (const bf16_t*)y, bnp, relu, M, C, rpb, part, (bf16_t*)gm);
-        else
-            hipLaunchKernelGGL((bn_bwd_reduce_kernel<half_t, 1024>), dim3(nblk), dim3(1024), 1024 * 16 * sizeof(float), s, (const half_t*)dout, (const half_t*)dout1,
-                               (const half_t*)dout2, (const half_t*)out, (const half_t*)y, bnp, relu, M, C, rpb, part, (half_t*)gm);
+        if (dtype == SDE_BF16) SDE_BN_REDUCE(bf16_t, 1024, 1024 * 16 * sizeof(float));
+        else SDE_BN_REDUCE(half_t, 1024, 1024 * 16 * sizeof(float));
     } else
-    DISPATCH_T(dtype,
-               hipLaunchKernelGGL(bn_bwd_reduce_kernel<float>, dim3(nblk), dim3(256), lds, s, (const float*)dout, (const float*)dout1, (const float*)dout2, (const float*)out, (const float*)y, bnp, relu, M, C, rpb, part, (float*)gm),
-               hipLaunchKernelGGL(bn_bwd_reduce_kernel<bf16_t>, dim3(nblk), dim3(256), lds, s, (const bf16_t*)dout, (const bf16_t*)dout1, (const bf16_t*)dout2, (const bf16_t*)out, (const bf16_t*)y, bnp, relu, M, C, rpb, part, (bf16_t*)gm),
-               hipLaunchKernelGGL(bn_bwd_reduce_kernel<half_t>, dim3(nblk), dim3(256), lds, s, (const half_t*)dout, (const half_t*)dout1, (const half_t*)dout2, (const half_t*)out, (const half_t*)y, bnp, relu, M, C, rpb, part, (half_t*)gm));
+        DISPATCH_T(dtype, SDE_BN_REDUCE(float, 256, lds), SDE_BN_REDUCE(bf16_t, 256, lds), SDE_BN_REDUCE(half_t, 256, lds));
+#undef SDE_BN_REDUCE
     SDE_CHECK_LAUNCH("sde_bn_bwd/reduce");
     const void* dz = gm ? gm : dout;
     if (g_bn_fuse && SDE_IS16(dtype) && C % 64 == 0 && nblk <= BNFA_MAX_ROWS) {
@@ -1354,6 +1452,29 @@
                hipLaunchKernelGGL(bn_bwd_apply_kernel<half_t>, dim3(nb), dim3(256), 0, s, (const half_t*)dz, (const half_t*)y, bnp, coef, M, C, (half_t*)dy));
     SDE_CHECK_LAUNCH("sde_bn_bwd/apply");
     return SDE_OK;
+}
+
+}
+
+extern "C" {
+
+int sde_bn_bwd(const void* dout, const void* dout1, const void* dout2, const void* out, const void* y, const float* bnp, const float* gamma, int relu,
+               long M, int C, int dtype, float* part, float* coef, float* dgamma, float* dbeta, int accumulate_params, void* gm, void* dy,
+               sde_stream_t stream) {
+    (void)gamma;
+    return bn_bwd_impl("sde_bn_bwd", dout, dout1, dout2, out, y, bnp, relu, M, C, dtype, part, coef, dgamma, dbeta, accumulate_params, gm, dy, nullptr, stream);
+}
+
+int sde_bn_bwd_pooled(const void* pool_d0, const void* pool_d1, const uint8_t* pool_idx, int B, int H, int W, const void* dout1, const void* dout2,
+                      const void* out, const void* y, const float* bnp, int relu, int C, int dtype, float* part, float* coef, float* dgamma, float* dbeta,
+                      int accumulate_params, void* gm, void* dy, sde_stream_t stream) {
+    const int V = SDE_IS16(dtype) ? 8 : 4;
+    SDE_CHECK_ARG(pool_d0 && pool_idx && gm && B > 0 && H > 1 && W > 1 && C > 0 && C % V == 0, "sde_bn_bwd_pooled: bad argument");
+    const long M = (long)B * H * W;
+    SDE_CHECK_ARG(M * (C / V) < (1L << 31), "sde_bn_bwd_pooled: more than 2^31 sixteen-byte groups");
+    const PoolSrc ps = {pool_d1, pool_idx, H, W, (H - 1) / 2 + 1, (W - 1) / 2 + 1};
+    return bn_bwd_impl("sde_bn_bwd_pooled", pool_d0, dout1, dout2, out, y, bnp, relu, M, C, dtype, part, coef, dgamma, dbeta, accumulate_params, gm, dy, &ps,
+                       stream);
 }
 
 int sde_bn_bwd_from_part(const float* part, int rows, const void* gm, const void* y, const float* bnp, long M, int C, int dtype, float* coef,
@@ -1412,10 +1533,12 @@
     SDE_CHECK_ARG(dout && idx && dx && B > 0 && H > 1 && W > 1 && C % V == 0, "sde_maxpool_bwd: bad argument");
     const int OH = (H + 2 - 3) / 2 + 1, OW = (W + 2 - 3) / 2 + 1;
     hipStream_t s = (hipStream_t)stream;
-    const int nb = grid_for((long)B * H * W * (C / V));
-    DISPATCH_T(dtype, hipLaunchKernelGGL(maxpool_bwd_kernel<float>, dim3(nb), dim3(256), 0, s, (const float*)dout, (const float*)dout1, idx, B, H, W, C, OH, OW, (float*)dx),
-               hipLaunchKernelGGL(maxpool_bwd_kernel<bf16_t>, dim3(nb), dim3(256), 0, s, (const bf16_t*)dout, (const bf16_t*)dout1, idx, B, H, W, C, OH, OW, (bf16_t*)dx),
-               hipLaunchKernelGGL(maxpool_bwd_kernel<half_t>, dim3(nb), dim3(256), 0, s, (const half_t*)dout, (const half_t*)dout1, idx, B, H, W, C, OH, OW, (half_t*)dx));
+    const long items = (long)B * H * W * (C / V);
+    const int nb = grid_for(items) < 2048 ? grid_for(items) : 2048;
+#define SDE_POOL_BWD(T, I) hipLaunchKernelGGL((maxpool_bwd_kernel<T, I>), dim3(nb), dim3(256), 0, s, (const T*)dout, (const T*)dout1, idx, B, H, W, C, OH, OW, (T*)dx)
+    if (items < (1L << 31)) DISPATCH_T(dtype, SDE_POOL_BWD(float, unsigned), SDE_POOL_BWD(bf16_t, unsigned), SDE_POOL_BWD(half_t, unsigned));
+    else DISPATCH_T(dtype, SDE_POOL_BWD(float, long), SDE_POOL_BWD(bf16_t, long), SDE_POOL_BWD(half_t, long));
+#undef SDE_POOL_BWD
     SDE_CHECK_LAUNCH("sde_maxpool_bwd");
     return SDE_OK;
 }
diff --git a/simpledepthestimation_amd/hip/nn.py b/simpledepthestimation_amd/hip/nn.py
--- a/simpledepthestimation_amd/hip/nn.py
+++ b/simpledepthestimation_amd/hip/nn.py
@@ -54,6 +54,7 @@
     "sde_bn_finalize_apply": ([_P, _I, _I, _LG, _P, _P, _P, _P, _F, _F, _P, _P, _P, _I, _I, _P, _P], c_int),
     "sde_reduce_num_blocks": ([_LG, _I], c_int),
     "sde_bn_bwd": ([_P, _P, _P, _P, _P, _P, _P, _I, _LG, _I, _I, _P, _P, _P, _P, _I, _P, _P, _P], c_int),
+    "sde_bn_bwd_pooled": ([_P, _P, _P, _I, _I, _I, _P, _P, _P, _P, _P, _I, _I, _I, _P, _P, _P, _P, _I, _P, _P, _P], c_int),
     "sde_maxpool_fwd": ([_P, _I, _I, _I, _I, _I, _P, _P, _P], c_int),
     "sde_depth_head_bias_blocks": ([_I, _I, _I], c_int),
     "sde_depth_head_bwd_bias": ([_P, _P, _I, _I, _I, _I, _F, _F, _I, _I, _P, _P, _P, _I, _P], c_int),
@@ -212,6 +213,8 @@
         self.res_grad = {}
         self.head_slot = {}
         self.head_done = {}
+        self.pool_in = {}
+        self.pool_grad = {}
 
     @staticmethod
     def _put(d, cap, t, ent):
@@ -265,9 +268,29 @@
         self.head_done = {k: v for k, v in self.head_done.items() if v != id(bias)}
         return len(self.head_done) < n
 
+    def put_pool_in(self, outs, y):
+        self.pool_grad.clear()
+        self._put(self.pool_in, 64, outs[0], (tuple(weakref.ref(o) for o in outs), y.data_ptr()))
+
+    def take_pool_in(self, x):
+        ent = self.pool_in.get(x.data_ptr())
+        if ent is None or not any(r() is x for r in ent[0]):
+            return None
+        return self.pool_in.pop(x.data_ptr())[1]
+
+    def put_pool_grad(self, g, ent):
+        self._put(self.pool_grad, 16, g, ent)
+
+    def take_pool_grad(self, g):
+        return self.pool_grad.pop(g.data_ptr(), None) if self.pool_grad else None
+
+    def pool_grad_pending(self, y_ptr):
+        return any(e[0] == y_ptr for e in self.pool_grad.values())
+
     def end_phase(self):
         self.res_grad.clear()
         self.bn_part.clear()
+        self.pool_grad.clear()
 
 
 _HANDOVER = _Handovers()
@@ -611,6 +634,8 @@
 FUSE_BN_FINALIZE = True
 BNBWD_FUSED = True
 BNBWD_HITS = 0
+POOLBWD_FUSED = True
+POOLBWD_HITS = 0
 RESBN_FUSED = os.environ.get("SDE_RESBN", "1") != "0"
 RESBN_HITS = 0
 _NO_PHASE = WGradReducer(defer=False)
@@ -928,7 +953,11 @@
         if training and relu and residual is not None and n_out == 2 and dt != torch.float32 and C % 64 == 0 and ctx.needs_input_grad[0] and BNBWD_FUSED and RESBN_FUSED:
             _HANDOVER.put_bn_out(out, y, bnp, res=True)
             ctx.res_tag = out.data_ptr()
-        return aliases(out, n_out)
+        outs = aliases(out, n_out)
+        if (training and relu and residual is None and n_out == 2 and y.dim() == 4 and dt != torch.float32 and C % 64 == 0 and ctx.needs_input_grad[0]
+                and POOLBWD_FUSED):
+            _HANDOVER.put_pool_in(outs, y)
+        return outs
 
     @staticmethod
     def backward(ctx, *douts):
@@ -971,6 +1000,24 @@
             return dy, None, dgamma, dbeta, None, None, (gm if has_res else None), None, None, None, None, None
         part = torch.empty(lib.sde_reduce_num_blocks(M, C) + REDUCE_ROWS, C, 2, device=dev)
         gm = torch.empty_like(y) if (relu or len(grads) > 1) else None
+        pooled = [(k, e) for k, e in ((k, _HANDOVER.take_pool_grad(g)) for k, g in enumerate(grads)) if e is not None]
+        if pooled:
+            k, (y_ptr, p0, p1, pidx, pshape) = pooled[0]
+            if not (len(pooled) == 1 and y_ptr == y.data_ptr() and relu and not has_res and tuple(y.shape) == pshape and p0.dtype == dt and len(grads) <= 2):
+                raise L.SdeHipError("BatchNorm backward: a max-pool gradient that was handed over instead of computed arrived at a BatchNorm it was not "
+                                    "formed for (hip.nn.POOLBWD_FUSED = False selects the separate max-pool backward)")
+            global POOLBWD_HITS
+            POOLBWD_HITS += 1
+            other = grads[1 - k] if len(grads) == 2 else None
+            L.check(lib.sde_bn_bwd_pooled(L.ptr(p0), L.ptr(p1), L.ptr(pidx), pshape[0], pshape[1], pshape[2], L.ptr(other), None, None, L.ptr(y), L.ptr(bnp),
+                                          1, C, dtype_code(dt), L.ptr(part), L.ptr(coef), L.ptr(dgamma), L.ptr(dbeta), int(direct), L.ptr(gm), L.ptr(dy),
+                                          L.stream()), "sde_bn_bwd_pooled")
+            if direct:
+                dgamma = dbeta = None
+            return dy, None, dgamma, dbeta, None, None, None, None, None, None, None, None
+        if _HANDOVER.pool_grad_pending(y.data_ptr()):
+            raise L.SdeHipError("BatchNorm backward: the max-pool behind this layer handed its gradient over, but it did not arrive here as it was returned "
+                                "(hip.nn.POOLBWD_FUSED = False selects the separate max-pool backward)")
         d0, d1, d2 = (grads + [None, None])[:3]
         L.check(lib.sde_bn_bwd(L.ptr(d0), L.ptr(d1), L.ptr(d2), L.ptr(out), L.ptr(y), L.ptr(bnp), L.ptr(gamma), int(relu), M, C, dtype_code(dt), L.ptr(part),
                                L.ptr(coef), L.ptr(dgamma), L.ptr(dbeta), int(direct), L.ptr(gm), L.ptr(dy), L.stream()), "sde_bn_bwd")
@@ -997,6 +1044,7 @@
         L.check(L.lib().sde_maxpool_fwd(L.ptr(x.contiguous()), B, H, W, C, dtype_code(x.dtype), L.ptr(out), L.ptr(idx), L.stream()), "sde_maxpool_fwd")
         ctx.save_for_backward(idx)
         ctx.shape = (B, H, W, C)
+        ctx.pool_tag = _HANDOVER.take_pool_in(x) if (POOLBWD_FUSED and ctx.needs_input_grad[0]) else None
         return aliases(out, n_out)
 
     @staticmethod
@@ -1008,6 +1056,9 @@
             return None, None
         d0, d1 = grads
         dx = torch.empty(B, H, W, C, device=d0.device, dtype=d0.dtype)
+        if ctx.pool_tag is not None:
+            _HANDOVER.put_pool_grad(dx, (ctx.pool_tag, d0, d1, idx, (B, H, W, C)))
+            return dx, None
         L.check(L.lib().sde_maxpool_bwd_sum(L.ptr(d0), L.ptr(d1), L.ptr(idx), B, H, W, C, dtype_code(d0.dtype), L.ptr(dx), L.stream()), "sde_maxpool_bwd_sum")
         return dx, None
 
```

After: 1921 images/s. Within noise of the previous version (-0.5%).
